# j-wilson/GPflowPILCO

Hardware: AMD Instinct MI355X
Metric: moment_matched_rollout_step_elements_per_sec (higher is better)
Workload: dtype f32; 1 GPU; C3 (BASELINE configs[2]): N=2000 d=8 D=8 H=40 fp32 drift moment-match step / closed rollout; recipe=baseline: BASELINE.md recipe: lengthscales log-U[0.3,3], GP-prior targets, fresh mu~U[0,1]^d / Sigm~; N=2000, d=8, D=8, H=40, B_per_gpu=256, B_total=256, B_this_rank=256, parallelism=dp1 over B (weak), recipe=baseline, steps_requested=418, diag_pairs=f64, offdiag_pairs=f32

## Files before the change

gpflowpilco_amd/_lib.py:

```python
from __future__ import annotations

import ctypes as C
import os

_HERE = os.path.dirname(os.path.abspath(__file__))
LIB_PATH = os.environ.get("GPFLOWPILCO_MM_LIB") or os.path.join(_HERE, "libgpflowpilco_mm.so")

MM_F32, MM_F64 = 0, 1
MM_DMAX = 32
MM_M_ALIGN = 128
MM_FULL_OUTPUT_COV = 1
MM_MODEL_UNCERTAINTY = 2
MM_FORCE_GENERIC = 4
MM_STAGE_DIAG = 8
MM_STAGE_OFFDIAG = 16
MM_STAGE_FINALIZE = 32
MM_FORCE_WORST_TIER = 64
MM_WORKSPACE_CURRENT = 128
MM_FORCE_ROUTE = 256
MM_NO_ROUTE = 512
MM_SUMS_CURRENT = 1024

ERRORS = {
    -1: "MM_E_ARG: NULL pointer or non-positive size",
    -2: "MM_E_DIM: input dimension d exceeds MM_DMAX=32 or unsupported shape",
    -3: "MM_E_DTYPE: dtype must be MM_F32 or MM_F64",
    -4: "MM_E_WORKSPACE: workspace/packed buffer too small",
    -5: "MM_E_NO_C: model_uncertainty requested but the model was packed without C",
    -6: "MM_E_STATE: Euler update / closed rollout needs d == L and a full output covariance",
}

SIGNATURES = {
    "mm_abi_version": (C.c_int, []),
    "mm_packed_model_bytes": (C.c_size_t, [C.c_int] * 5),
    "mm_pack_model": (C.c_int, [C.c_void_p, C.c_size_t, C.c_int, C.c_int, C.c_int, C.c_int]
                      + [C.c_void_p] * 6 + [C.c_void_p]),
    "mm_pack_perm": (C.c_int, [C.c_void_p, C.c_size_t, C.c_int, C.c_int, C.c_int, C.c_int, C.c_void_p, C.c_void_p]),
    "mm_workspace_bytes": (C.c_size_t, [C.c_int] * 6),
    "mm_moment_match": (C.c_int, [C.c_void_p, C.c_size_t, C.c_int, C.c_int, C.c_int, C.c_int, C.c_int,
                                  C.c_void_p, C.c_void_p, C.c_int, C.c_double,
                                  C.c_void_p, C.c_void_p, C.c_void_p,
                                  C.c_void_p, C.c_size_t, C.c_void_p, C.c_void_p]),
    "mm_q_forward": (C.c_int, [C.c_void_p, C.c_size_t, C.c_int, C.c_int, C.c_int, C.c_int, C.c_int,
                               C.c_void_p, C.c_void_p, C.c_int,
                               C.c_void_p, C.c_void_p, C.c_void_p,
                               C.c_void_p, C.c_size_t, C.c_void_p, C.c_void_p]),
    "mm_Q_reduce_forward": (C.c_int, [C.c_void_p, C.c_size_t, C.c_int, C.c_int, C.c_int, C.c_int, C.c_int,
                                      C.c_int, C.c_double, C.c_void_p,
                                      C.c_void_p, C.c_size_t, C.c_void_p]),
    "mm_euler_update": (C.c_int, [C.c_int, C.c_int, C.c_int, C.c_double] + [C.c_void_p] * 8),
    "mm_expected_cost": (C.c_int, [C.c_int, C.c_int, C.c_int] + [C.c_void_p] * 6),
    "mm_offdiag_stats": (C.c_int, [C.c_void_p, C.c_size_t, C.c_int, C.c_int, C.c_int, C.c_int, C.c_int, C.c_int,
                                   C.c_void_p, C.c_size_t, C.c_void_p, C.c_void_p]),
    "mm_route_estimates": (C.c_int, [C.c_void_p, C.c_size_t, C.c_int, C.c_int, C.c_int, C.c_int, C.c_int, C.c_int,
                                     C.c_void_p, C.c_size_t, C.c_void_p, C.c_void_p]),
    "mm_compose_workspace_bytes": (C.c_size_t, [C.c_int] * 4),
    "mm_rollout_composed": (C.c_int, [C.c_void_p, C.c_size_t, C.c_int, C.c_int, C.c_int,
                                      C.c_void_p, C.c_size_t, C.c_int, C.c_int,
                                      C.c_int, C.c_int, C.c_int, C.c_double, C.c_int, C.c_int, C.POINTER(C.c_int32),
                                      C.c_double, C.c_double, C.c_void_p, C.c_void_p,
                                      C.c_void_p, C.c_void_p, C.c_void_p, C.c_void_p, C.c_void_p,
                                      C.c_void_p, C.c_size_t, C.c_void_p, C.c_size_t, C.c_void_p, C.c_size_t,
                                      C.c_void_p, C.c_void_p]),
    "mm_compose_nd_workspace_bytes": (C.c_size_t, [C.c_int] * 5),
    "mm_rollout_composed_nd": (C.c_int, [C.c_void_p, C.c_size_t, C.c_int, C.c_int, C.c_int,
                                         C.c_void_p, C.c_size_t, C.c_int, C.c_int,
                                         C.c_int, C.c_int, C.c_int, C.c_double, C.c_int, C.c_int, C.POINTER(C.c_int32),
                                         C.c_int, C.POINTER(C.c_double), C.POINTER(C.c_double), C.c_void_p, C.c_void_p,
                                         C.c_void_p, C.c_void_p, C.c_void_p, C.c_void_p, C.c_void_p,
                                         C.c_void_p, C.c_size_t, C.c_void_p, C.c_size_t, C.c_void_p, C.c_size_t,
                                         C.c_void_p, C.c_void_p]),
    "mm_compose_tape_bytes": (C.c_size_t, [C.c_int] * 6),
    "mm_rollout_composed_taped": (C.c_int, [C.c_void_p, C.c_size_t, C.c_int, C.c_int, C.c_int,
                                            C.c_void_p, C.c_size_t, C.c_int, C.c_int,
                                            C.c_int, C.c_int, C.c_int, C.c_double, C.c_int, C.c_int, C.POINTER(C.c_int32),
                                            C.c_double, C.c_double, C.c_void_p, C.c_void_p,
                                            C.c_void_p, C.c_void_p, C.c_void_p,
                                            C.c_void_p, C.c_size_t, C.c_void_p, C.c_size_t, C.c_void_p, C.c_size_t,
                                            C.c_void_p, C.c_void_p]),
    "mm_compose_backward_workspace_bytes": (C.c_size_t, [C.c_int] * 4),
    "mm_policy_grad_bytes": (C.c_size_t, [C.c_int] * 3),
    "mm_rollout_composed_backward": (C.c_int, [C.c_void_p, C.c_size_t, C.c_int, C.c_int, C.c_int,
                                               C.c_void_p, C.c_size_t, C.c_int, C.c_int,
                                               C.c_int, C.c_int, C.c_int, C.c_double, C.c_int, C.c_int, C.POINTER(C.c_int32),
                                               C.c_double, C.c_double, C.c_void_p, C.c_void_p,
                                               C.c_void_p, C.c_size_t, C.c_void_p,
                                               C.c_void_p, C.c_void_p, C.c_void_p,
                                               C.c_void_p, C.c_size_t, C.c_void_p, C.c_size_t,
                                               C.c_void_p, C.c_void_p]),
    "mm_rollout_composed_backward_seeded": (C.c_int, [C.c_void_p, C.c_size_t, C.c_int, C.c_int, C.c_int,
                                                      C.c_void_p, C.c_size_t, C.c_int, C.c_int,
                                                      C.c_int, C.c_int, C.c_int, C.c_double, C.c_int, C.c_int, C.POINTER(C.c_int32),
                                                      C.c_double, C.c_double, C.c_void_p, C.c_void_p,
                                                      C.c_void_p, C.c_size_t, C.c_void_p, C.c_void_p, C.c_void_p,
                                                      C.c_void_p, C.c_void_p, C.c_void_p,
                                                      C.c_void_p, C.c_size_t, C.c_void_p, C.c_size_t,
                                                      C.c_void_p, C.c_void_p]),
    "mm_compose_tape_bytes_nd": (C.c_size_t, [C.c_int] * 7),
    "mm_rollout_composed_taped_nd": (C.c_int, [C.c_void_p, C.c_size_t, C.c_int, C.c_int, C.c_int,
                                               C.c_void_p, C.c_size_t, C.c_int, C.c_int,
                                               C.c_int, C.c_int, C.c_int, C.c_double, C.c_int, C.c_int, C.POINTER(C.c_int32),
                                               C.c_int, C.POINTER(C.c_double), C.POINTER(C.c_double), C.c_void_p, C.c_void_p,
                                               C.c_void_p, C.c_void_p, C.c_void_p,
                                               C.c_void_p, C.c_size_t, C.c_void_p, C.c_size_t, C.c_void_p, C.c_size_t,
                                               C.c_void_p, C.c_void_p]),
    "mm_compose_backward_workspace_bytes_nd": (C.c_size_t, [C.c_int] * 6),
    "mm_policy_grad_bytes_nd": (C.c_size_t, [C.c_int] * 4),
    "mm_rollout_composed_backward_nd": (C.c_int, [C.c_void_p, C.c_size_t, C.c_int, C.c_int, C.c_int,
                                                  C.c_void_p, C.c_size_t, C.c_int, C.c_int,
                                                  C.c_int, C.c_int, C.c_int, C.c_double, C.c_int, C.c_int, C.POINTER(C.c_int32),
                                                  C.c_int, C.POINTER(C.c_double), C.POINTER(C.c_double), C.c_void_p, C.c_void_p,
                                                  C.c_void_p, C.c_size_t, C.c_void_p,
                                                  C.c_void_p, C.c_void_p, C.c_void_p,
                                                  C.c_void_p, C.c_size_t, C.c_void_p, C.c_size_t,
                                                  C.c_void_p, C.c_void_p]),
    "mm_rollout_composed_backward_nd_seeded": (C.c_int, [C.c_void_p, C.c_size_t, C.c_int, C.c_int, C.c_int,
                                                         C.c_void_p, C.c_size_t, C.c_int, C.c_int,
                                                         C.c_int, C.c_int, C.c_int, C.c_double, C.c_int, C.c_int, C.POINTER(C.c_int32),
                                                         C.c_int, C.POINTER(C.c_double), C.POINTER(C.c_double), C.c_void_p, C.c_void_p,
                                                         C.c_void_p, C.c_size_t, C.c_void_p, C.c_void_p, C.c_void_p,
                                                         C.c_void_p, C.c_void_p, C.c_void_p,
                                                         C.c_void_p, C.c_size_t, C.c_void_p, C.c_size_t,
                                                         C.c_void_p, C.c_void_p]),
    "mm_compose_nd_mixed_workspace_bytes": (C.c_size_t, [C.c_int] * 6),
    "mm_rollout_composed_nd_mixed": (C.c_int, [C.c_void_p, C.c_size_t, C.c_int, C.c_int, C.c_int,
                                               C.c_void_p, C.c_size_t, C.c_int, C.c_int,
                                               C.c_int, C.c_int, C.c_int, C.c_double, C.c_int, C.c_int, C.POINTER(C.c_int32),
                                               C.c_int, C.POINTER(C.c_double), C.POINTER(C.c_double), C.c_void_p, C.c_void_p,
                                               C.c_void_p, C.c_void_p, C.c_void_p, C.c_void_p, C.c_void_p,
                                               C.c_void_p, C.c_size_t, C.c_void_p, C.c_size_t, C.c_void_p, C.c_size_t,
                                               C.c_void_p, C.c_void_p, C.c_void_p, C.c_void_p]),
    "mm_compose_tape_bytes_nd_mixed": (C.c_size_t, [C.c_int] * 8),
    "mm_rollout_composed_taped_nd_mixed": (C.c_int, [C.c_void_p, C.c_size_t, C.c_int, C.c_int, C.c_int,
                                                     C.c_void_p, C.c_size_t, C.c_int, C.c_int,
                                                     C.c_int, C.c_int, C.c_int, C.c_double, C.c_int, C.c_int, C.POINTER(C.c_int32),
                                                     C.c_int, C.POINTER(C.c_double), C.POINTER(C.c_double), C.c_void_p, C.c_void_p,
# ... 134 lines not shown
```

gpflowpilco_amd/csrc/mm_common.h:

```cpp
#pragma once
#include <stddef.h>
#include <stdint.h>
#include "../../include/gpflowpilco_mm.h"

static inline size_t mm_align_up(size_t x, size_t a) { return (x + a - 1) / a * a; }
static inline int mm_round_up_int(int x, int a) { return (x + a - 1) / a * a; }
static inline size_t mm_elem_size(int dtype) { return dtype == MM_F64 ? 8 : 4; }

#define MM_ISTAGE_NO_ROUTE (1 << 20)
#define MM_ISTAGE_ROUTE (1 << 21)
#define MM_ISTAGE_NO_M56 (1 << 22)
#define MM_ISTAGE_OLD_OFFDIAG (1 << 23)
#define MM_ISTAGE_OLD_SPOLY56 (1 << 24)
#define MM_ISTAGE_OLD_DIAG_MAP (1 << 25)

#define MM_PW_KERNELS 3

static inline int mm_num_pairs(int L, int flags) {
  return (flags & MM_FULL_OUTPUT_COV) ? L * (L + 1) / 2 : L;
}

static inline int mm_moment_deg(int d) { return d <= 8 ? 4 : 2; }
static inline long long mm_binom(int n, int k) {
  if (k < 0 || k > n) return 0;
  long long r = 1;
  for (int i = 1; i <= k; ++i) r = r * (n - k + i) / i;
  return r;
}
static inline int mm_mono_count(int n, int d) { return (int)mm_binom(d + n - 1, n); }
static inline int mm_mono_offset(int n, int d) { int o = 0; for (int m = 0; m < n; ++m) o += mm_mono_count(m, d); return o; }
static inline size_t mm_rank_table_entries(int d) {
  const int dk = d <= 8 ? 8 : 32, deg = mm_moment_deg(d);
  size_t n = 0, p = 1;
  for (int k = 1; k <= deg; ++k) { p *= dk; n += p; }
  return n;
}
static inline int mm_moment_cols(int d) { return mm_round_up_int(mm_mono_offset(mm_moment_deg(d) + 1, d), 16); }
static inline int mm_moment56_off5(int d) { return d <= 8 ? mm_round_up_int(mm_mono_count(4, d), 128) : 0; }
static inline int mm_moment56_off6(int d) { return d <= 8 ? mm_moment56_off5(d) + mm_round_up_int(mm_mono_count(5, d), 128) : 0; }
static inline int mm_moment56_cols(int d) { return d <= 8 ? mm_moment56_off6(d) + mm_round_up_int(mm_mono_count(6, d), 128) : 0; }
struct MMTab56 { int ins[6], last[6], n_i16, mult2, mult3, n_f32; size_t bytes; };
static inline MMTab56 mm_tab56(int d) {
  MMTab56 t;
  int o = 0;
  for (int m = 0; m < 6; ++m) { t.ins[m] = o; o += mm_mono_count(m, d) * 8; }
  for (int k = 0; k < 6; ++k) { t.last[k] = o; o += mm_mono_count(k, d); }
  t.n_i16 = mm_round_up_int(o, 8);
  t.mult2 = 0; t.mult3 = mm_mono_count(2, d); t.n_f32 = mm_mono_count(2, d) + mm_mono_count(3, d);
  t.bytes = (size_t)t.n_i16 * 2 + (size_t)t.n_f32 * 4;
  return t;
}

struct MMModelLayout {
  int Mp, Kz, nd8, KMp;
  size_t Z64;
  size_t Zt64;
  size_t zbar;
  size_t ls2;
  size_t var;
  size_t meanc;
  size_t beta64;
  size_t Zc64;
  size_t Zc;
  size_t Zs3;
  size_t Zm;
  size_t zmax2;
  size_t rtab;
  size_t Zq2;
  size_t Zm56;
  size_t tab56;
  size_t perm;
  size_t skey;
  size_t zt2;
  size_t Cm;
  size_t total;
};
#define MM_SORT_MIN_M 256

static inline MMModelLayout mm_model_layout(int L, int M, int d, int dtype, int with_C) {
  MMModelLayout o;
  const size_t es = mm_elem_size(dtype), A = 256;
  o.Mp = mm_round_up_int(M, MM_M_ALIGN);
  o.Kz = mm_round_up_int(d, 2);
  o.nd8 = (d + 7) / 8;
  o.KMp = mm_moment_cols(d);
  size_t off = 0;
  o.Z64 = off;    off = mm_align_up(off + (size_t)L * M * d * 8, A);
  o.Zt64 = off;   off = mm_align_up(off + (size_t)L * d * o.Mp * 8, A);
  o.zbar = off;   off = mm_align_up(off + (size_t)L * d * 8, A);
  o.ls2 = off;    off = mm_align_up(off + (size_t)L * d * 8, A);
  o.var = off;    off = mm_align_up(off + (size_t)L * 8, A);
  o.meanc = off;  off = mm_align_up(off + (size_t)L * 8, A);
  o.beta64 = off; off = mm_align_up(off + (size_t)L * M * 8, A);
  o.Zc64 = off;   off = mm_align_up(off + (size_t)L * o.Mp * o.Kz * 8, A);
  o.Zc = o.Zc64;
  if (dtype != MM_F64) { o.Zc = off; off = mm_align_up(off + (size_t)L * o.Mp * o.Kz * es, A); }
  o.Zs3 = off;
  if (dtype != MM_F64) off = mm_align_up(off + (size_t)L * o.Mp * 24 * o.nd8 * 2, A);
  o.Zm = off;
  if (dtype != MM_F64) off = mm_align_up(off + (size_t)L * o.Mp * o.KMp * 8, A);
  o.zmax2 = off;  off = mm_align_up(off + (size_t)L * 8, A);
  o.rtab = off;   off = mm_align_up(off + mm_rank_table_entries(d) * 2, A);
  o.Zq2 = off;
  if (dtype != MM_F64 && d <= 8) off = mm_align_up(off + (size_t)L * (o.Mp / 32) * 8192, A);
  o.Zm56 = off;
  if (dtype != MM_F64 && d <= 8) off = mm_align_up(off + (size_t)L * 2 * mm_moment56_cols(d) * o.Mp * 2, A);
  o.tab56 = off;
  if (dtype != MM_F64 && d <= 8) off = mm_align_up(off + mm_tab56(d).bytes, A);
  o.perm = off;   off = mm_align_up(off + (size_t)L * o.Mp * 4, A);
  o.skey = off;   off = mm_align_up(off + (size_t)L * o.Mp * 8, A);
  o.zt2 = off;    off = mm_align_up(off + (size_t)L * (o.Mp / 32) * 4, A);
  o.Cm = off;
  if (with_C) off = mm_align_up(off + (size_t)L * o.Mp * o.Mp * 8, A);
  o.total = off;
  return o;
}

#define MM_MOM_SPLIT 2
#ifndef MM_COLLAPSE_BOUND2
#define MM_COLLAPSE_BOUND2 0.25f
#endif
#define MM_C6_X5_2 (1.0f / 256.0f)
#define MM_C6_X4_2 (1.0f / 1600.0f)
#define MM_C6_MAX 0.25f
#define MM_C6_C0 1.666663289e-01f
#define MM_C6_C1 4.166659713e-02f
#define MM_C6_C2 8.350561373e-03f
#define MM_C6_C3 1.391559141e-03f
#define MM_C6_SYS2 6.33e-6f
#define MM_C6_POLY_F64(x_) (((x_) * (x_)) * (x_) * fma(fma(fma((double)MM_C6_C3, (x_), (double)MM_C6_C2), (x_), (double)MM_C6_C1), (x_), (double)MM_C6_C0))
#ifndef MM_TIER1_DIV
#define MM_TIER1_DIV 20
#endif
#if MM_TIER1_DIV == 16
#define MM_TIER1_MAX 0.0625f
#define MM_REM1_C0 1.666936278e-01f
#define MM_REM1_C1 4.167173430e-02f
#elif MM_TIER1_DIV == 20
#define MM_TIER1_MAX 0.05f
#define MM_REM1_C0 1.666839272e-01f
#define MM_REM1_C1 4.166988656e-02f
#elif MM_TIER1_DIV == 24
#define MM_TIER1_MAX 0.041666668f
#define MM_REM1_C0 1.666786522e-01f
#define MM_REM1_C1 4.166889191e-02f
#elif MM_TIER1_DIV == 32
#define MM_TIER1_MAX 0.03125f
#define MM_REM1_C0 1.666734070e-01f
#define MM_REM1_C1 4.166791216e-02f
#else
#error "MM_TIER1_DIV must be 16, 20, 24 or 32"
#endif
#define MM_INSIDE_BOUND2 (0.998f * MM_C6_MAX * MM_C6_MAX)
#ifndef MM_ROUTE_TOL
#define MM_ROUTE_TOL 3.0e-4
#endif
#define MM_ROUTE_CSPLIT 8
static inline int mm_route_ncc(int NS, int npanel) { int n = NS / npanel; return n < 1 ? 1 : (n > MM_ROUTE_CSPLIT ? MM_ROUTE_CSPLIT : n); }
#define MM_EXP_CAP_F64 700.0
#define MM_EXP_CAP_F32 80.0f
#define MM_GEN_ROWS 64
#define MM_GEN_COLS 256
#define MM_PANEL_ROWS 256
__host__ __device__ inline int mm_mfma_groups(int Mp) { return (Mp + MM_PANEL_ROWS - 1) / MM_PANEL_ROWS * (MM_PANEL_ROWS / 64); }
__host__ __device__ inline int mm_f32p_list_off(int L) { return 4 + 2 * L; }
#define MM_F64_TILE 64

struct MMWorkspaceLayout {
  int Mp, P, Po, NS;
  size_t pairmat;
  size_t latmat;
  size_t rho1;
  size_t w64;
  size_t q64;
  size_t w;
  size_t lq;
  size_t rowD;
  size_t colD;
  size_t qhR;
  size_t qhC;
  size_t rowO;
  size_t colO;
  size_t f1raw;
  size_t whR;
  size_t whC;
  size_t mom;
  size_t amax;
  size_t amaxc;
  size_t gflag;
  size_t gperm;
  size_t s12;
  size_t gmax2;
  size_t partB;
  size_t partC;
  size_t mu64;
  size_t estO;
  size_t rlist;
  size_t rcount;
  size_t rflag;
  size_t wsp;
  size_t mom56;
  size_t estS;
  size_t ilist;
  size_t plist;
  size_t s56;
  size_t f1s;
  size_t Sffs;
  size_t crs;
  size_t total;
};

static inline MMWorkspaceLayout mm_workspace_layout(int B, int L, int M, int d, int dtype, int flags) {
  MMWorkspaceLayout o;
  const size_t es = mm_elem_size(dtype), A = 256;
  o.Mp = mm_round_up_int(M, MM_M_ALIGN);
  o.P = mm_num_pairs(L, flags);
  o.Po = o.P - L;
  const int nrb = (o.Mp + MM_GEN_ROWS - 1) / MM_GEN_ROWS;
  const int ncb = (o.Mp + MM_GEN_COLS - 1) / MM_GEN_COLS;
  const int nt = o.Mp / MM_F64_TILE;
  int ns = nrb * ncb;
  if (nt * (nt + 1) / 2 > ns) ns = nt * (nt + 1) / 2;
  if (dtype == MM_F64 && o.Po > 0 && nt * nt > ns) ns = nt * nt;
  o.NS = ns;
  size_t off = 0;
  o.pairmat = off; off = mm_align_up(off + (size_t)B * o.P * (d * d + 1) * 8, A);
  o.latmat = off;  off = mm_align_up(off + (size_t)B * L * (2 * d * d + 2) * 8, A);
  o.rho1 = off;    off = mm_align_up(off + (size_t)B * L * o.Mp * 8, A);
  o.w64 = off;     off = mm_align_up(off + (size_t)B * L * o.Mp * 8, A);
  o.q64 = off;     off = mm_align_up(off + (size_t)B * L * o.Mp * 8, A);
  o.w = o.w64;
  o.lq = off;      off = mm_align_up(off + (size_t)B * L * o.Mp * 8, A);
  o.rowD = off;    off = mm_align_up(off + (size_t)B * L * o.Mp * 8, A);
  o.colD = off;    off = mm_align_up(off + (size_t)B * L * (d + 1) * o.Mp * 8, A);
  o.qhR = off;     off = mm_align_up(off + (size_t)B * L * o.Mp * 8, A);
  o.qhC = off;     off = mm_align_up(off + (size_t)B * L * o.Mp * 8, A);
  const size_t nrow = dtype == MM_F64 ? 1 : (size_t)(d + 1), ncol = dtype == MM_F64 ? (size_t)(d + 1) : 1;
  o.rowO = off;    off = mm_align_up(off + (size_t)B * o.Po * nrow * o.Mp * es, A);
  o.colO = off;    off = mm_align_up(off + (size_t)B * o.Po * ncol * o.Mp * es, A);
  o.f1raw = off;   off = mm_align_up(off + (size_t)B * L * 8, A);
  const size_t nwh = dtype == MM_F64 ? 0 : (size_t)B * o.Po * o.Mp;
  o.whR = off;     off = mm_align_up(off + nwh * 8, A);
  o.whC = off;     off = mm_align_up(off + nwh * 8, A);
  o.mom = off;     off = mm_align_up(off + (dtype == MM_F64 ? 0 : (size_t)B * o.Po * 2 * MM_MOM_SPLIT * mm_moment_cols(d) * 8), A);
  o.amax = off;    off = off + (size_t)B * o.Po * 4;
  o.amaxc = off;   off = mm_align_up(off + (size_t)B * o.Po * 4, A);
  o.gflag = off;   off = mm_align_up(off + (dtype == MM_F64 ? 0 : (size_t)B * o.Po * (o.Mp / 64)), A);
  o.gmax2 = off;   off = mm_align_up(off + (dtype == MM_F64 ? 0 : (size_t)B * o.Po * (o.Mp / 64) * 4), A);
  o.gperm = off;   off = mm_align_up(off + (dtype == MM_F64 || L < 2 ? 0 : ((size_t)L * (L - 1) * B + 3 * L) * 4), A);
  o.s12 = off;     off = mm_align_up(off + (size_t)B * o.Po * 8, A);
  o.partB = off;   off = mm_align_up(off + (size_t)B * o.P * o.NS * 8, A);
  o.partC = off;   off = mm_align_up(off + (size_t)B * L * o.NS * 8, A);
  const size_t nro = dtype == MM_F64 ? 0 : (size_t)B * o.Po;
  o.mu64 = off;    off = mm_align_up(off + (size_t)B * d * 8, A);
  o.estO = off;    off = mm_align_up(off + nro * ((o.Mp + MM_PANEL_ROWS - 1) / MM_PANEL_ROWS) * 4, A);
  o.rlist = off;   off = mm_align_up(off + nro * 4, A);
  o.rcount = off;  off = mm_align_up(off + 16, A);
  o.rflag = off;   off = mm_align_up(off + nro * 4, A);
  const size_t n56 = (dtype == MM_F64 || d > 8) ? 0 : (size_t)B * o.Po;
  o.wsp = off;     off = mm_align_up(off + n56 * 4 * o.Mp * 2, A);
  o.mom56 = off;   off = mm_align_up(off + n56 * 2 * mm_moment56_cols(d) * 4, A);
  o.estS = off;    off = mm_align_up(off + n56 * 4, A);
  o.s56 = off;     off = mm_align_up(off + n56 * 8, A);
  o.ilist = off;   off = mm_align_up(off + n56 * 4 + 16, A);
  o.plist = off;   off = mm_align_up(off + (n56 ? (n56 + mm_f32p_list_off(L)) * 4 : 0), A);
  o.f1s = off;     off = mm_align_up(off + (size_t)B * L * es, A);
  o.Sffs = off;    off = mm_align_up(off + (size_t)B * L * L * es, A);
  o.crs = off;     off = mm_align_up(off + (size_t)B * d * L * es, A);
  o.total = off;
  return o;
}
```

gpflowpilco_amd/csrc/mm_kernels.hip:

```cpp
#include <hip/hip_runtime.h>
#include <math.h>
#include "mm_common.h"
#include "mm_cost.h"
#include "mm_dev.h"
#include "mm_mono.h"

#include <mutex>
#include <unordered_map>
#include "mm_fork.h"

#define MM_ABI_VERSION 2

namespace {
struct MMForkKey {
  int dev; hipStream_t stream;
  bool operator==(const MMForkKey& o) const { return dev == o.dev && stream == o.stream; }
};
struct MMForkKeyHash {
  size_t operator()(const MMForkKey& k) const { return std::hash<const void*>()((const void*)k.stream) * 31u + (size_t)k.dev; }
};
std::mutex g_fork_mu;
std::unordered_map<MMForkKey, MMFork*, MMForkKeyHash> g_forks;

MMFork* mm_fork_lookup(hipStream_t stream, bool create) {
// ... 107 lines not shown
  const double* Z = (const double*)(packed + lay.Z64);
  double* zbar = (double*)(packed + lay.zbar) + (size_t)a * d;
  double* ls2 = (double*)(packed + lay.ls2) + (size_t)a * d;
  double* Zc64 = (double*)(packed + lay.Zc64) + (size_t)a * lay.Mp * lay.Kz;
  T* Zc = (T*)(packed + lay.Zc) + (size_t)a * lay.Mp * lay.Kz;
  __shared__ double red[4];
  __shared__ double zb[MM_DMAX];
  for (int k = 0; k < d; ++k) {
    double s = 0.0;
    for (int m = tid; m < M; m += 256) s += Z[((size_t)a * M + m) * d + k];
    s = mm_block_sum256(s, red);
    if (tid == 0) zb[k] = s / (double)M;
  }
  __syncthreads();
  if (tid < d) { zbar[tid] = zb[tid]; const double l = ls[a * d + tid]; ls2[tid] = l * l; }
  if (tid == 0) {
    ((double*)(packed + lay.var))[a] = var[a];
    ((double*)(packed + lay.meanc))[a] = mean_c ? mean_c[a] : 0.0;
  }
  {
    double* Zt = (double*)(packed + lay.Zt64) + (size_t)a * d * lay.Mp;
    for (int idx = tid; idx < d * lay.Mp; idx += 256) {
      const int k = idx / lay.Mp, m = idx - k * lay.Mp;
      Zt[idx] = m < M ? Z[((size_t)a * M + m) * d + k] : 0.0;
    }
  }
  for (int idx = tid; idx < lay.Mp * lay.Kz; idx += 256) {
    const int m = idx / lay.Kz, k = idx - m * lay.Kz;
    double v = 0.0;
    if (m < M && k < d) v = Z[((size_t)a * M + m) * d + k] - zb[k];
    Zc64[idx] = v;
    if (sizeof(T) != 8) Zc[idx] = (T)v;
  }
  if (sizeof(T) != 8) {
    double* Zm = (double*)(packed + lay.Zm) + (size_t)a * lay.Mp * lay.KMp;
    const int deg = d <= 8 ? 4 : 2;
    const int ncol = mm_mono_off(deg + 1, d);
    for (int idx = tid; idx < lay.Mp * lay.KMp; idx += 256) {
      const int m = idx / lay.KMp, c = idx - m * lay.KMp;
      double v = 0.0;
      if (m < M && c < ncol) {
        int n = 0;
        while (mm_mono_off(n + 1, d) <= c) ++n;
        int k[4] = {0, 0, 0, 0};
        mm_mono_unrank(c - mm_mono_off(n, d), n, k);
        v = 1.0;
        for (int t = 0; t < n; ++t) v *= Z[((size_t)a * M + m) * d + k[t]] - zb[k[t]];
      }
      Zm[idx] = v;
    }
    if (a == 0) {
      short* rt = (short*)(packed + lay.rtab);
      const int lb = d <= 8 ? 3 : 5;
      size_t base = 0;
      for (int kk = 1; kk <= deg; ++kk) {
        const int sz = 1 << (lb * kk);
        for (int idx = tid; idx < sz; idx += 256) {
          int dg[4] = {0, 0, 0, 0};
          bool in = true;
          for (int t = 0; t < kk; ++t) { dg[t] = (idx >> (lb * t)) & ((1 << lb) - 1); in = in && dg[t] < d; }
          for (int i = 1; i < kk; ++i)
            for (int j = i; j > 0 && dg[j - 1] > dg[j]; --j) { const int t2 = dg[j]; dg[j] = dg[j - 1]; dg[j - 1] = t2; }
          rt[base + idx] = in ? (short)mm_mono_rank(dg, kk) : (short)-1;
        }
        base += sz;
      }
    }
  }
  {
    double zm2 = 0.0;
    for (int m = tid; m < M; m += 256) {
      double s2 = 0.0;
      for (int k = 0; k < d; ++k) { const double v = Z[((size_t)a * M + m) * d + k] - zb[k]; s2 += v * v; }
      zm2 = s2 > zm2 ? s2 : zm2;
    }
#pragma unroll
    for (int off = 32; off > 0; off >>= 1) { const double o = __shfl_down(zm2, off, 64); zm2 = o > zm2 ? o : zm2; }
    __syncthreads();
    if ((tid & 63) == 0) red[tid >> 6] = zm2;
    __syncthreads();
    if (tid == 0) ((double*)(packed + lay.zmax2))[a] = fmax(fmax(red[0], red[1]), fmax(red[2], red[3]));
    __syncthreads();
    float* zt2 = (float*)(packed + lay.zt2) + (size_t)a * (lay.Mp / 32);
    for (int t = tid; t < lay.Mp / 32; t += 256) {
      double mx = 0.0;
      for (int j = 0; j < 32; ++j) {
        const int m = t * 32 + j;
        if (m >= M) break;
        double s2 = 0.0;
        for (int k = 0; k < d; ++k) { const double v = Z[((size_t)a * M + m) * d + k] - zb[k]; s2 += v * v; }
        mx = s2 > mx ? s2 : mx;
      }
      zt2[t] = (float)(mx * 1.000001);
    }
  }
  if (sizeof(T) != 8) {
    unsigned short* Zs3 = (unsigned short*)(packed + lay.Zs3) + (size_t)a * lay.Mp * 24 * lay.nd8;
    const int kw = 8 * lay.nd8;
    for (int idx = tid; idx < lay.Mp * kw; idx += 256) {
      const int m = idx / kw, k = idx - m * kw;
      float v = 0.0f;
      if (m < M && k < d) v = (float)(Z[((size_t)a * M + m) * d + k] - zb[k]);
      const __bf16 h = (__bf16)v;
      float r = v - (float)h;
      const __bf16 mm = (__bf16)r;
      r -= (float)mm;
      const __bf16 l = (__bf16)r;
      unsigned short* o = Zs3 + ((size_t)(m >> 5) * 3 * 32 + (m & 31)) * kw + k;
      o[0] = __builtin_bit_cast(unsigned short, h);
      o[32 * kw] = __builtin_bit_cast(unsigned short, mm);
      o[64 * kw] = __builtin_bit_cast(unsigned short, l);
    }
    if (d <= 8) {
      unsigned short* Zq = (unsigned short*)(packed + lay.Zq2) + (size_t)a * (lay.Mp / 32) * 4096;
      const int nslot = 1 + d + d * (d + 1) / 2;
      for (int idx = tid; idx < (lay.Mp / 32) * 2048; idx += 256) {
        int r = idx;
        const int t = r & 7; r >>= 3;
        const int ln = r & 63; r >>= 6;
        const int nb = r & 1; r >>= 1;
        const int s2 = r & 1; r >>= 1;
        const int ct = r;
        const int slot = 32 * nb + (ln & 31), hh = ln >> 5;
        const int m = 32 * ct + 16 * s2 + 8 * (t >> 2) + 4 * hh + (t & 3);
        float v = 0.0f;
        if (m < M && slot < nslot) {
          if (slot == 0) v = 1.0f;
          else if (slot <= d) v = (float)(Z[((size_t)a * M + m) * d + slot - 1] - zb[slot - 1]);
          else {
            int qq = slot - 1 - d, l0 = 0;
            while (qq >= d - l0) { qq -= d - l0; ++l0; }
            const int l1 = l0 + qq;
            v = (float)((Z[((size_t)a * M + m) * d + l0] - zb[l0]) * (Z[((size_t)a * M + m) * d + l1] - zb[l1]));
          }
        }
        const __bf16 h = (__bf16)v;
        const __bf16 lo = (__bf16)(v - (float)h);
        unsigned short* o = Zq + ((((size_t)(ct * 2 + s2) * 2 + nb) * 2) * 64 + ln) * 8 + t;
        o[0] = __builtin_bit_cast(unsigned short, h);
        o[512] = __builtin_bit_cast(unsigned short, lo);
      }
    }
  }
}

__global__ void k_pack_C(char* packed, MMModelLayout lay, int L, int M, const double* __restrict__ C) {
  const int j = blockIdx.x * 256 + threadIdx.x, i = blockIdx.y, a = blockIdx.z;
  if (j >= lay.Mp) return;
  double* Cm = (double*)(packed + lay.Cm) + ((size_t)a * lay.Mp + i) * lay.Mp;
  const int* pm = (const int*)(packed + lay.perm) + (size_t)a * lay.Mp;
  double v = 0.0;
  if (i < M && j < M) v = C[((size_t)a * M + pm[i]) * M + pm[j]];
  Cm[j] = v;
}

template <typename T>
__global__ __launch_bounds__(192) void k_prep(const double* __restrict__ ls2, const double* __restrict__ var,
                                              int L, int d, int P,
                                              const T* __restrict__ mu, const T* __restrict__ Sigma,
                                              double* __restrict__ pairmat, double* __restrict__ latmat,
                                              unsigned int* __restrict__ amax, int32_t* status, int pairs_pass) {
  extern __shared__ double smem[];
  const int dp = d + 1, msz = d * dp;
  double* Sg = smem;
  double* A0 = Sg + msz;
  double* A1 = A0 + msz;
  double* A2 = A1 + msz;
  double* Tm = A2 + msz;
  double* Y = Tm + msz;
  __shared__ double lds3[3];
  __shared__ int okw[3];
  const int tid = threadIdx.x, nt = blockDim.x, wv = tid >> 6;
  const int item = pairs_pass == 0 ? P + blockIdx.x : blockIdx.x, b = blockIdx.y;
  bool ok = true;
  const T* Sb = Sigma + (size_t)b * d * d;
  for (int idx = tid; idx < d * d; idx += nt) {
// ... 179 lines not shown
        maha = fma(z[i], t, maha);
        rv = fma(z[i], te, rv);
      };
      if constexpr (QREG) {
        int t = 0;
#pragma unroll
        for (int i = 0; i < DK; ++i) {
          const double pd = Pr[QREG ? t : 0] * z[i], ed = Er[QREG ? t : 0] * z[i];
          ++t;
          double tp = 0.0, te = 0.0;
#pragma unroll
          for (int k = i + 1; k < DK; ++k, ++t) { tp = fma(Pr[QREG ? t : 0], z[k], tp); te = fma(Er[QREG ? t : 0], z[k], te); }
          maha = fma(z[i], fma(2.0, tp, pd), maha);
          rv = fma(z[i], fma(2.0, te, ed), rv);
        }
      } else {
#pragma unroll 2
        for (int i = 0; i < DK; ++i) row(i);
      }
      lqv = lognorm - 0.5 * maha;
      qv = exp(lqv);
      wv = bt * qv;
      acc_f += wv;
#pragma unroll
      for (int k = 0; k < DK; ++k) acc_s[k] += wv * z[k];
      if (q_out) q_out[((size_t)b * L + a) * M + perm[(size_t)a * Mp + m]] = (T)qv;
    }
    wb64[m] = wv;
    qb64[m] = qv;
    r1[m] = rv;
    lqb[m] = lqv;
  };
  {
    double zA[DK], zB[DK], bA, bB;
    loadz(tid, zA, bA);
    for (int m = tid; m < Mp; m += 512) {
      loadz(m + 256 < Mp ? m + 256 : m, zB, bB);
      chunk(m, zA, bA);
      if (m + 256 >= Mp) break;
      loadz(m + 512 < Mp ? m + 512 : m + 256, zA, bA);
      chunk(m + 256, zB, bB);
    }
  }
  __shared__ double red9[4][DK + 1];
  {
    double v[DK + 1];
#pragma unroll
    for (int k = 0; k < DK; ++k) v[k] = acc_s[k];
    v[DK] = acc_f;
#pragma unroll
    for (int k = 0; k <= DK; ++k) {
#pragma unroll
      for (int off = 32; off > 0; off >>= 1) v[k] += __shfl_down(v[k], off, 64);
    }
    if ((tid & 63) == 0) {
#pragma unroll
      for (int k = 0; k <= DK; ++k) red9[tid >> 6][k] = v[k];
    }
  }
  __syncthreads();
  if (tid <= DK) sv[tid] = (red9[0][tid] + red9[1][tid]) + (red9[2][tid] + red9[3][tid]);
  __syncthreads();
  if (tid == 0) { f1[(size_t)b * L + a] = (T)(sv[DK] + meanc[a]); f1raw[(size_t)b * L + a] = sv[DK]; }
  if (tid < d) {
    double s = 0.0;
    for (int k = 0; k < d; ++k) s += Pa[tid * DK + k] * sv[k];
    cross[((size_t)b * d + tid) * L + a] = (T)s;
  }
}

template <typename T, int DK>
__global__ __launch_bounds__(256) void k_pairvec(const double* __restrict__ Zt64, const double* __restrict__ zbar,
                                                 const double* __restrict__ ls2, int L, int M, int Mp, int d, int P,
                                                 const T* __restrict__ mu, const double* __restrict__ pairmat,
                                                 const double* __restrict__ rho1,
                                                 double* __restrict__ rowD, double* __restrict__ colD,
                                                 T* __restrict__ rowO, T* __restrict__ colO,
                                                 const double* __restrict__ w64, double* __restrict__ whR,
                                                 double* __restrict__ whC, unsigned int* __restrict__ amax,
                                                 const double* __restrict__ q64, double* __restrict__ qhR,
                                                 double* __restrict__ qhC, int with_unc, int nblk,
                                                 const double* __restrict__ lq, const double* __restrict__ beta64,
                                                 const double* __restrict__ zmax2, unsigned short* __restrict__ ,
                                                 unsigned char* __restrict__ , float* __restrict__ , int , int p0) {
  static_assert(DK > 8, "d <= 8 takes k_pairvec_reg");
  const int p = p0 + (int)blockIdx.y, b = blockIdx.z, tid = threadIdx.x;
  int a, a2;
  mm_decode_pair(p, L, a, a2);
  const double* r1a = rho1 + ((size_t)b * L + a) * Mp;
  const double* r1b = rho1 + ((size_t)b * L + a2) * Mp;
  __shared__ __align__(16) double Ts[DK * DK];
  __shared__ double vecs[7][DK];
  __shared__ int rcs;
  const double* pm = pairmat + ((size_t)b * P + p) * (d * d + 1);
  for (int idx = tid; idx < DK * DK; idx += 256) {
    const int i = idx / DK, k = idx - i * DK;
    const bool in = i < d && k < d;
    Ts[idx] = in ? pm[i * d + k] * ls2[a * d + i] * ls2[a2 * d + k] : 0.0;
  }
  if (tid < DK) {
    const int k = tid < d ? tid : 0;
    const double mv = (double)mu[(size_t)b * d + k];
    const double la = ls2[a * d + k], lb = ls2[a2 * d + k];
    vecs[0][tid] = tid < d ? mv : 0.0;
    vecs[1][tid] = tid < d ? 1.0 / la : 0.0;
    vecs[2][tid] = tid < d ? 1.0 / lb : 0.0;
    vecs[3][tid] = tid < d ? (mv - zbar[a2 * d + k]) / lb : 0.0;
    vecs[4][tid] = tid < d ? (mv - zbar[a * d + k]) / la : 0.0;
  }
  __syncthreads();
  const double cst = pm[d * d];
  const bool diag = p < L;
  const int Po = P - L;
  const bool f32off = !diag && sizeof(T) == 4;
  if (f32off) {
    if (tid < DK) {
      double t = 0.0;
      for (int k = 0; k < DK; ++k) t = fma(Ts[tid * DK + k], vecs[4][k], t);
      vecs[5][tid] = t;
    }
    __syncthreads();
    if (tid == 0) {
      double sa2 = 0.0, c00 = 0.0;
      for (int i = 0; i < DK; ++i) { const double sa = vecs[5][i] * vecs[2][i]; sa2 = fma(sa, sa, sa2); c00 = fma(vecs[5][i], vecs[3][i], c00); }
      const bool rc = sa2 * zmax2[a2] <= MM_RECENTRE_CMAX * MM_RECENTRE_CMAX;
      rcs = rc ? 1 : 0;
      vecs[6][0] = rc ? c00 : 0.0;
      if (!rc) for (int i = 0; i < DK; ++i) vecs[5][i] = 0.0;
    }
    __syncthreads();
  }
  const bool recentred = f32off ? rcs != 0 : true;
  T* rO = rowO + ((size_t)b * Po + (f32off ? p - L : 0)) * (size_t)(d + 1) * Mp;
  T* cO = colO + ((size_t)b * Po + (f32off ? p - L : 0)) * Mp;
  double* hR = whR + ((size_t)b * Po + (f32off ? p - L : 0)) * Mp;
  double* hC = whC + ((size_t)b * Po + (f32off ? p - L : 0)) * Mp;
  double* raD = rowD + ((size_t)b * L + (diag ? p : 0)) * Mp;
  double* cbD = colD + ((size_t)b * L + (diag ? p : 0)) * (size_t)(d + 1) * Mp;
  T* raO = rowO + ((size_t)b * Po + (diag ? 0 : p - L)) * Mp;
  T* cbO = colO + ((size_t)b * Po + (diag ? 0 : p - L)) * (size_t)(d + 1) * Mp;
  float a2max = 0.0f;
  for (int mblk = blockIdx.x; mblk < nblk; mblk += gridDim.x) {
    const int m = mblk * 256 + tid;
    if (m >= Mp) continue;
    typedef const __attribute__((address_space(3))) double* lds_cptr;
    lds_cptr vl = (lds_cptr)&vecs[0][0], tl = (lds_cptr)Ts;
    asm volatile("" : "+v"(vl), "+v"(tl));
    double zr[DK], zc[DK];
#pragma unroll
    for (int k = 0; k < DK; ++k) {
      const int kk = k < d ? k : 0;
      const double vr = Zt64[((size_t)a * d + kk) * Mp + m];
      const double vc = Zt64[((size_t)a2 * d + kk) * Mp + m];
      zr[k] = (m < M) ? (vr - vl[k]) * vl[DK + k] : 0.0;
      zc[k] = (m < M) ? (vc - vl[k]) * vl[2 * DK + k] : 0.0;
    }
    const double r1r = r1a[m], r1c = r1b[m];
    const int mc = m < M ? m : M - 1;
    const double lqr = lq[((size_t)b * L + a) * Mp + m], lqc = lq[((size_t)b * L + a2) * Mp + m];
    const double btr = beta64[(size_t)a * M + mc], btc = beta64[(size_t)a2 * M + mc];
    double tA = 0.0, tg = 0.0, corrA = 0.0, corrg = 0.0;
    double asq = 0.0, cj = vl[6 * DK];
#pragma unroll 2
    for (int i = 0; i < DK; ++i) {
      double u = 0.0, v = 0.0;
#pragma unroll
      for (int k = 0; k < DK; ++k) {
        const double t = tl[i * DK + k];
        u = fma(t, zr[k], u);
        v = fma(t, zc[k], v);
      }
      tA = fma(zr[i], u, tA);
      tg = fma(zc[i], v, tg);
      corrA = fma(vl[3 * DK + i], u, corrA);
      corrg = fma(vl[4 * DK + i], v, corrg);
      const double t0i = f32off ? vl[5 * DK + i] : 0.0;
      cj = fma(t0i, zc[i], cj);
      const double av = (u + t0i) * vl[2 * DK + i], gv = v * vl[DK + i];
      asq = fma(av, av, asq);
      if (i < d) {
        if (f32off) rO[(size_t)i * Mp + m] = (T)av;
        else if (diag) cbD[(size_t)i * Mp + m] = gv;
        else cbO[(size_t)i * Mp + m] = (T)gv;
      }
    }
    const double rho_q = (m < M) ? r1r - tA : 0.0;
    const double gam_q = (m < M) ? r1c - tg : 0.0;
    if (f32off) {
      a2max = fmaxf(a2max, (float)asq * 1.000001f);
      double whr = 0.0, whc = 0.0;
      if (m < M) {
        whr = btr * exp(fmin(lqr - 0.5 * rho_q + cst - corrA, (double)MM_EXP_CAP_F32));
        whc = btc * exp(fmin(lqc - 0.5 * gam_q - cj, (double)MM_EXP_CAP_F32));
      }
      rO[(size_t)d * Mp + m] = (T)whr;
      cO[m] = (T)whc;
      hR[m] = whr;
      hC[m] = whc;
    } else {
      const double rowv = -0.5 * rho_q;
      const double colv = (m < M) ? -0.5 * gam_q + cst - corrg : 0.0;
      if (diag) {
        raD[m] = rowv; cbD[(size_t)d * Mp + m] = colv;
        const size_t qi = ((size_t)b * L + p) * Mp + m;
        const double u = (m < M) ? (with_unc ? 1.0 : btr) : 0.0;
        qhR[qi] = u * exp(fmin(lqr + rowv, MM_EXP_CAP_F64));
        qhC[qi] = u * exp(fmin(lqr + colv, MM_EXP_CAP_F64));
      } else { raO[m] = (T)rowv; cbO[(size_t)d * Mp + m] = (T)colv; }
    }
  }
  if (f32off && amax) {
#pragma unroll
    for (int off = 32; off > 0; off >>= 1) a2max = fmaxf(a2max, __shfl_down(a2max, off, 64));
    if ((tid & 63) == 0) atomicMax(amax + (size_t)b * Po + (p - L), recentred ? __float_as_uint(a2max) : MM_AMAX_NOT_RECENTRED);
  }
}

template <typename T, int DK, int MODE>
__device__ __forceinline__ void mm_pairvec_reg_body(const double* __restrict__ Zt64, const double* __restrict__ zbar,
                                                    const double* __restrict__ ls2, int L, int M, int Mp, int d, int P,
                                                    const T* __restrict__ mu, const double* __restrict__ pairmat,
                                                    const double* __restrict__ rho1,
                                                    double* __restrict__ rowD, double* __restrict__ colD,
                                                    T* __restrict__ rowO, T* __restrict__ colO,
                                                    const double* __restrict__ w64, double* __restrict__ whR,
                                                    double* __restrict__ whC, unsigned int* __restrict__ amax,
                                                    const double* __restrict__ q64, double* __restrict__ qhR,
                                                    double* __restrict__ qhC, int with_unc, int nblk, int a, int a2,
                                                    double (*vecs)[DK], const double* __restrict__ lq,
                                                    const double* __restrict__ beta64, int p, const double* __restrict__ zmax2,
                                                    unsigned short* __restrict__ wsp, unsigned char* __restrict__ gflag, float* __restrict__ gmax2,
                                                    int allow) {
  constexpr bool diag = MODE == 0;
  const int b = blockIdx.z, tid = threadIdx.x;
  const int Po = P - L;
  const double* zA = Zt64 + (size_t)a * d * Mp;
  const double* zB = Zt64 + (size_t)a2 * d * Mp;
  const double* r1a = rho1 + ((size_t)b * L + a) * Mp;
  const double* r1b = rho1 + ((size_t)b * L + a2) * Mp;
  const double* wa = lq + ((size_t)b * L + a) * Mp;
  const double* wb = lq + ((size_t)b * L + a2) * Mp;
  const double* ba = beta64 + (size_t)a * M;
  const double* bb = beta64 + (size_t)a2 * M;
  struct Ops { double zr[DK], zc[diag ? 1 : DK], r1r, r1c, wr, wc, br, bc; };
  auto load_ops = [&](int mblk, Ops& o) {
    int m = mblk * 256 + tid;
    m = m < Mp ? m : Mp - 1;
#pragma unroll
    for (int k = 0; k < DK; ++k) {
      const unsigned off = (unsigned)((k < d ? k : 0) * Mp + m);
      o.zr[k] = zA[off];
      if constexpr (!diag) o.zc[k] = zB[off];
    }
    o.r1r = r1a[m];
    o.wr = wa[m];
    const int mb = m < M ? m : M - 1;
    o.br = ba[mb];
    if constexpr (!diag) { o.r1c = r1b[m]; o.wc = wb[m]; o.bc = bb[mb]; }
  };
  Ops oA, oB;
  load_ops(blockIdx.x, oA);
  const double* pm = pairmat + ((size_t)b * P + p) * (d * d + 1);
  constexpr int NT = DK * (DK + 1) / 2;
  double Tr[NT];
  auto tsym = [](int i, int k) { return i <= k ? i * DK - i * (i - 1) / 2 + (k - i) : k * DK - k * (k - 1) / 2 + (i - k); };
  {
    const int ln = tid & 63, li = ln / DK, lk = ln - li * DK;
    const bool lin = li < d && lk < d && ln < DK * DK;
    const double mine = lin ? pm[li * d + lk] * ls2[a * d + li] * ls2[a2 * d + lk] : 0.0;
    const int mlo = __double2loint(mine), mhi = __double2hiint(mine);
#pragma unroll
    for (int i = 0; i < DK; ++i)
#pragma unroll
      for (int k = i; k < DK; ++k) {
        double t = __hiloint2double(__builtin_amdgcn_readlane(mhi, i * DK + k), __builtin_amdgcn_readlane(mlo, i * DK + k));
        asm volatile("" : "+v"(t));
        Tr[tsym(i, k)] = t;
      }
  }
  if (tid < DK) {
    const int k = tid < d ? tid : 0;
    const double mv = (double)mu[(size_t)b * d + k];
    const double la = ls2[a * d + k], lb = ls2[a2 * d + k];
    vecs[0][tid] = tid < d ? mv : 0.0;
    vecs[1][tid] = tid < d ? 1.0 / la : 0.0;
    vecs[2][tid] = tid < d ? 1.0 / lb : 0.0;
    vecs[3][tid] = tid < d ? (mv - zbar[a2 * d + k]) / lb : 0.0;
    vecs[4][tid] = tid < d ? (mv - zbar[a * d + k]) / la : 0.0;
  }
  __syncthreads();
  bool recentred = true;
  if constexpr (MODE == 0) {
    double h2 = 0.0, t0[DK];
#pragma unroll
    for (int i = 0; i < DK; ++i) {
      double t = 0.0;
#pragma unroll
      for (int k = 0; k < DK; ++k) t = fma(Tr[tsym(i, k)], vecs[4][k], t);
      t0[i] = t;
      const double hi = t * vecs[1][i];
      h2 = fma(hi, hi, h2);
    }
    recentred = h2 * zmax2[a] <= MM_RECENTRE_CMAX * MM_RECENTRE_CMAX;
    if (tid == 0) {
#pragma unroll
      for (int i = 0; i < DK; ++i) vecs[5][i] = recentred ? t0[i] : 0.0;
    }
    __syncthreads();
  }
  if constexpr (MODE == 1) {
    double sa2 = 0.0, c00 = 0.0, t0[DK];
#pragma unroll
    for (int i = 0; i < DK; ++i) {
      double t = 0.0;
#pragma unroll
      for (int k = 0; k < DK; ++k) t = fma(Tr[tsym(i, k)], vecs[4][k], t);
      t0[i] = t;
      const double sa = t * vecs[2][i];
      sa2 = fma(sa, sa, sa2);
      c00 = fma(t, vecs[3][i], c00);
    }
    recentred = sa2 * zmax2[a2] <= MM_RECENTRE_CMAX * MM_RECENTRE_CMAX;
    if (tid == 0) {
#pragma unroll
      for (int i = 0; i < DK; ++i) vecs[5][i] = recentred ? t0[i] : 0.0;
      vecs[6][0] = recentred ? c00 : 0.0;
    }
    __syncthreads();
  }
  const double cst = pm[d * d];
  float a2max = 0.0f;
  float a2cmax = 0.0f, a2in = 0.0f;
  const bool cancoll = MODE == 1 && allow && recentred;
  const double zm2c = MODE == 1 ? zmax2[a2] : 0.0;
  typedef const __attribute__((address_space(3))) double* lds_cptr;
  auto rowi = [&](int i) { return (unsigned)((i < d ? i : d) * Mp); };
  const unsigned rowd = (unsigned)(d * Mp);

  auto body = [&](int mblk, const Ops& o) {
    const int m = mblk * 256 + tid;
    if (m >= Mp) return;
    lds_cptr vl = (lds_cptr)&vecs[0][0];
    asm volatile("" : "+v"(vl));
    const bool live = m < M;
    if constexpr (MODE == 0) {
      double* cbD = colD + ((size_t)b * L + p) * (size_t)(d + 1) * Mp;
      double* raD = rowD + ((size_t)b * L + p) * Mp;
      double* qR = qhR + ((size_t)b * L + p) * Mp;
      double* qC = qhC + ((size_t)b * L + p) * Mp;
      if (live) {
        double sv[DK];
#pragma unroll
        for (int k = 0; k < DK; ++k) sv[k] = (o.zr[k] - vl[k]) * vl[DK + k];
        double tq = 0.0, corr = 0.0, zh = 0.0;
#pragma unroll
        for (int i = 0; i < DK; ++i) {
          double u = 0.0;
#pragma unroll
          for (int k = 0; k < DK; ++k) u = fma(Tr[tsym(i, k)], sv[k], u);
          tq = fma(sv[i], u, tq);
          corr = fma(vl[4 * DK + i], u, corr);
          zh = fma(sv[i] + vl[4 * DK + i], vl[5 * DK + i], zh);
          cbD[rowi(i) + m] = (u + vl[5 * DK + i]) * vl[DK + i];
        }
        const double row0 = -0.5 * (o.r1r - tq);
        const double rowv = row0 - zh;
        const double colv = row0 + cst - corr;
        const double uw = with_unc ? 1.0 : o.br;
        raD[m] = rowv; cbD[rowd + m] = colv;
        qR[m] = uw * exp(fmin(o.wr + rowv, MM_EXP_CAP_F64)); qC[m] = uw * exp(fmin(o.wr + colv, MM_EXP_CAP_F64));
      } else {
#pragma unroll
        for (int i = 0; i < DK; ++i) cbD[rowi(i) + m] = 0.0;
        raD[m] = 0.0; cbD[rowd + m] = 0.0; qR[m] = 0.0; qC[m] = 0.0;
      }
    } else if constexpr (MODE == 1) {
      T* rO = rowO + ((size_t)b * Po + (p - L)) * (size_t)(d + 1) * Mp;
      T* cO = colO + ((size_t)b * Po + (p - L)) * Mp;
      double* hR = whR + ((size_t)b * Po + (p - L)) * Mp;
      double* hC = whC + ((size_t)b * Po + (p - L)) * Mp;
      double whr = 0.0, whc = 0.0;
      bool rowok = true;
      if (live) {
        double sr[DK], sc[DK];
        double cj = vl[6 * DK];
#pragma unroll
        for (int k = 0; k < DK; ++k) {
          const double muk = vl[k];
          sr[k] = (o.zr[k] - muk) * vl[DK + k]; sc[k] = (o.zc[k] - muk) * vl[2 * DK + k];
          cj = fma(vl[5 * DK + k], sc[k], cj);
        }
        double tA = 0.0, tg = 0.0, corrA = 0.0, asq = 0.0;
#pragma unroll
        for (int i = 0; i < DK; ++i) {
          double u = 0.0, vh = 0.0;
#pragma unroll
          for (int k = 0; k < DK; ++k) {
            const double t = Tr[tsym(i, k)];
            u = fma(t, sr[k], u);
            if (k > i) vh = fma(t, sc[k], vh);
          }
          tA = fma(sr[i], u, tA);
          tg = fma(sc[i], fma(2.0, vh, Tr[tsym(i, i)] * sc[i]), tg);
          const double av = (u + vl[5 * DK + i]) * vl[2 * DK + i];
          asq = fma(av, av, asq);
          corrA = fma(vl[3 * DK + i], u, corrA);
          rO[rowi(i) + m] = (T)av;
        }
        const float a2row = (float)asq * 1.000001f;
        a2max = fmaxf(a2max, a2row);
        rowok = mm_collapse_bound2(__float_as_uint(a2row), zm2c) <= MM_COLLAPSE_BOUND2;
        a2in = a2row;
        whr = o.br * exp(fmin(o.wr - 0.5 * (o.r1r - tA) + cst - corrA, (double)MM_EXP_CAP_F32));
        whc = o.bc * exp(fmin(o.wc - 0.5 * (o.r1c - tg) - cj, (double)MM_EXP_CAP_F32));
      } else {
#pragma unroll
        for (int i = 0; i < DK; ++i) rO[rowi(i) + m] = (T)0;
        a2in = 0.0f;
      }
      rO[rowd + m] = (T)whr; cO[m] = (T)whc; hR[m] = whr; hC[m] = whc;
      if (wsp) {
        const bool inner = cancoll && __all(rowok);
        float g2 = a2in;
#pragma unroll
        for (int off = 32; off > 0; off >>= 1) g2 = fmaxf(g2, __shfl_xor(g2, off, 64));
        if ((tid & 63) == 0) {
          const size_t gi = ((size_t)b * Po + (p - L)) * (size_t)(Mp / MM_GROUP_ROWS) + (m >> 6);
          gflag[gi] = inner ? 1 : 0;
          gmax2[gi] = g2;
        }
        if (inner) a2cmax = fmaxf(a2cmax, a2in);
        unsigned short* sp = wsp + ((size_t)b * Po + (p - L)) * 4 * (size_t)Mp + m;
        const float fr = inner ? (float)whr : 0.0f, fc = (float)whc;
        const __bf16 rh = (__bf16)fr, ch = (__bf16)fc;
        const __bf16 rm = (__bf16)(fr - (float)rh), cm = (__bf16)(fc - (float)ch);
        sp[0] = __builtin_bit_cast(unsigned short, rh); sp[Mp] = __builtin_bit_cast(unsigned short, rm);
        sp[2 * (size_t)Mp] = __builtin_bit_cast(unsigned short, ch); sp[3 * (size_t)Mp] = __builtin_bit_cast(unsigned short, cm);
      }
    } else {
      T* raO = rowO + ((size_t)b * Po + (p - L)) * Mp;
      T* cbO = colO + ((size_t)b * Po + (p - L)) * (size_t)(d + 1) * Mp;
      if (live) {
        double sr[DK], sc[DK];
#pragma unroll
        for (int k = 0; k < DK; ++k) { const double muk = vl[k]; sr[k] = (o.zr[k] - muk) * vl[DK + k]; sc[k] = (o.zc[k] - muk) * vl[2 * DK + k]; }
        double tA = 0.0, tg = 0.0, corrg = 0.0;
#pragma unroll
        for (int i = 0; i < DK; ++i) {
          double v = 0.0, uh = 0.0;
#pragma unroll
          for (int k = 0; k < DK; ++k) {
            const double t = Tr[tsym(i, k)];
            v = fma(t, sc[k], v);
            if (k > i) uh = fma(t, sr[k], uh);
          }
          tg = fma(sc[i], v, tg);
          tA = fma(sr[i], fma(2.0, uh, Tr[tsym(i, i)] * sr[i]), tA);
          corrg = fma(vl[4 * DK + i], v, corrg);
          cbO[rowi(i) + m] = (T)(v * vl[DK + i]);
        }
        raO[m] = (T)(-0.5 * (o.r1r - tA));
        cbO[rowd + m] = (T)(-0.5 * (o.r1c - tg) + cst - corrg);
      } else {
#pragma unroll
        for (int i = 0; i < DK; ++i) cbO[rowi(i) + m] = (T)0;
        raO[m] = (T)0; cbO[rowd + m] = (T)0;
      }
    }
  };

  const int step = (int)gridDim.x;
  for (int mblk = blockIdx.x; mblk < nblk; mblk += 2 * step) {
    load_ops(mblk + step < nblk ? mblk + step : mblk, oB);
    body(mblk, oA);
    if (mblk + step >= nblk) break;
    load_ops(mblk + 2 * step < nblk ? mblk + 2 * step : mblk + step, oA);
    body(mblk + step, oB);
  }
  if (MODE == 1 && amax) {
#pragma unroll
    for (int off = 32; off > 0; off >>= 1) a2max = fmaxf(a2max, __shfl_down(a2max, off, 64));
    if ((tid & 63) == 0) atomicMax(amax + (size_t)b * Po + (p - L), recentred ? __float_as_uint(a2max) : MM_AMAX_NOT_RECENTRED);
#pragma unroll
    for (int off = 32; off > 0; off >>= 1) a2cmax = fmaxf(a2cmax, __shfl_down(a2cmax, off, 64));
    if ((tid & 63) == 0 && a2cmax > 0.0f) atomicMax(amax + ((size_t)gridDim.z + b) * Po + (p - L), __float_as_uint(a2cmax));
  }
}

template <typename T, int DK>
__global__ __launch_bounds__(256, 2) void k_pairvec_reg(const double* __restrict__ Zt64, const double* __restrict__ zbar,
                                                        const double* __restrict__ ls2, int L, int M, int Mp, int d, int P,
                                                        const T* __restrict__ mu, const double* __restrict__ pairmat,
                                                        const double* __restrict__ rho1,
                                                        double* __restrict__ rowD, double* __restrict__ colD,
                                                        T* __restrict__ rowO, T* __restrict__ colO,
                                                        const double* __restrict__ w64, double* __restrict__ whR,
                                                        double* __restrict__ whC, unsigned int* __restrict__ amax,
                                                        const double* __restrict__ q64, double* __restrict__ qhR,
                                                        double* __restrict__ qhC, int with_unc, int nblk,
                                                        const double* __restrict__ lq, const double* __restrict__ beta64,
                                                        const double* __restrict__ zmax2, unsigned short* __restrict__ wsp,
                                                        unsigned char* __restrict__ gflag, float* __restrict__ gmax2, int allow, int p0) {
  static_assert(DK <= 8, "register form: d <= 8");
  __shared__ double vecs[7][DK];
  const int p = p0 + (int)blockIdx.y;
  int a, a2;
  mm_decode_pair(p, L, a, a2);
#define MM_PV_BODY(MODE_)                                                                                           \
  mm_pairvec_reg_body<T, DK, MODE_>(Zt64, zbar, ls2, L, M, Mp, d, P, mu, pairmat, rho1, rowD, colD, rowO, colO, w64, \
                                    whR, whC, amax, q64, qhR, qhC, with_unc, nblk, a, a2, vecs, lq, beta64, p, zmax2, wsp, gflag, gmax2, allow)
  if (p < L) MM_PV_BODY(0);
  else if (sizeof(T) == 4) MM_PV_BODY(1);
  else MM_PV_BODY(2);
#undef MM_PV_BODY
}

template <typename T, int DK, bool ROWVEC>
__global__ __launch_bounds__(256) void k_qred_generic(const T* __restrict__ Zc, int Kz, const double* __restrict__ Cm,
                                                      int L, int Mp, int d, int P, int NS, int ncb, int p0,
                                                      const T* __restrict__ w, const T* __restrict__ q,
                                                      const T* __restrict__ rowA, const T* __restrict__ colB,
                                                      double* __restrict__ partB, double* __restrict__ partC,
                                                      const unsigned char* __restrict__ gflag, const unsigned int* __restrict__ amaxc,
                                                      const double* __restrict__ zmax2) {
  const int cbk = blockIdx.x % ncb, rbk = blockIdx.x / ncb;
  const int lp = blockIdx.y, np = gridDim.y, p = p0 + lp, b = blockIdx.z, tid = threadIdx.x;
  int a, a2;
  mm_decode_pair(p, L, a, a2);
  const int j = cbk * MM_GEN_COLS + tid;
  const bool jv = j < Mp;
  const int jj = jv ? j : 0;
  const T* cb = ROWVEC ? colB + ((size_t)b * np + lp) * Mp
                       : colB + ((size_t)b * np + lp) * (size_t)(d + 1) * Mp;
  T g[DK];
#pragma unroll
  for (int k = 0; k < DK; ++k)
    g[k] = (k < d) ? (ROWVEC ? Zc[((size_t)a2 * Mp + jj) * Kz + k] : cb[(size_t)k * Mp + jj]) : (T)0;
  const T gam = ROWVEC ? (T)0 : cb[(size_t)d * Mp + jj];
  const T wj = jv ? (ROWVEC ? cb[jj] : w[((size_t)b * L + a2) * Mp + jj]) : (T)0;
  const bool withC = (Cm != nullptr) && (a == a2);
  const T qj = (withC && jv) ? q[((size_t)b * L + a2) * Mp + jj] : (T)0;
  const T* ra = ROWVEC ? rowA + ((size_t)b * np + lp) * (size_t)(d + 1) * Mp
                       : rowA + ((size_t)b * np + lp) * Mp;
  const T* wr = w + ((size_t)b * L + a) * Mp;
  const T* qr = q + ((size_t)b * L + a) * Mp;
  const T* zrow = Zc + (size_t)a * Mp * Kz;
  const int i0 = rbk * MM_GEN_ROWS;
  const int i1 = (i0 + MM_GEN_ROWS < Mp) ? i0 + MM_GEN_ROWS : Mp;
  T accB = (T)0;
  double sumB = 0.0, sumC = 0.0;
  const unsigned char* gf = (ROWVEC && gflag != nullptr && zmax2 != nullptr) ? gflag + ((size_t)b * np + lp) * (size_t)(Mp / MM_GROUP_ROWS) : nullptr;
  const bool icoll = gf != nullptr && mm_item_collapsed(amaxc[(size_t)b * np + lp]);
  for (int i = i0; i < i1; ++i) {
    const bool coll = icoll && gf[i >> 6] != 0;
    T delta = ROWVEC ? (T)0 : ra[i] + gam;
#pragma unroll
    for (int k = 0; k < DK; ++k)
      if (k < d) delta += (ROWVEC ? ra[(size_t)k * Mp + i] : zrow[(size_t)i * Kz + k]) * g[k];
    const double dd = fmin((double)delta, sizeof(T) == 8 ? MM_EXP_CAP_F64 : (double)MM_EXP_CAP_F32);
    const T e = ROWVEC ? (T)(expm1(dd) - dd - 0.5 * dd * dd - (coll ? MM_C6_POLY_F64(dd) : (icoll ? (double)MM_C6_C0 * dd * dd * dd : 0.0)))
                       : (T)expm1(dd);
    accB += (ROWVEC ? ra[(size_t)d * Mp + i] : wr[i]) * e;
    if (withC) {
      const double cij = Cm[((size_t)a * Mp + i) * Mp + jj];
      const double qi = (double)qr[i];
      sumC += cij * (qi * (double)e + qi);
    }
    if (((i - i0) & 15) == 15) { sumB += (double)accB; accB = (T)0; }
  }
  sumB += (double)accB;
  sumB *= (double)wj;
  sumC *= (double)qj;
  __shared__ double red[4];
  const double tb = mm_block_sum256(sumB, red);
  if (tid == 0) partB[((size_t)b * P + p) * NS + blockIdx.x] = tb;
  if (withC) {
    const double tc = mm_block_sum256(sumC, red);
    if (tid == 0) partC[((size_t)b * L + a) * NS + blockIdx.x] = tc;
  }
}

template <typename T>
__global__ __launch_bounds__(256) void k_finalize(const double* __restrict__ partB, const double* __restrict__ partC,
                                                  const double* __restrict__ var, int B, int L, int P, int NS,
                                                  int nsB_diag, int nsB_off, int nsC, int full, int with_unc,
                                                  double jitter, const double* __restrict__ f1raw,
                                                  const double* __restrict__ s12, const double* __restrict__ s56, int diag_factored,
                                                  const int* __restrict__ rflag, int ns_routed, T* __restrict__ Sff) {
  const int idx = blockIdx.x * 4 + (threadIdx.x >> 6), lane = threadIdx.x & 63;
  if (idx >= B * P) return;
  const int b = idx / P, p = idx - b * P;
  int a, a2;
  mm_decode_pair(p, L, a, a2);
// ... 125 lines not shown
  hipLaunchKernelGGL(k_pack_gather, dim3((M + 255) / 256, L), dim3(256), 0, s, packed, lay, M, d, Z, beta);
  MM_CHECK_LAUNCH();
  hipLaunchKernelGGL((k_pack_vectors<T>), dim3(L), dim3(256), 0, s, packed, lay, L, M, d, ls, var, mean_c);
  MM_CHECK_LAUNCH();
  if (sizeof(T) == 4 && d <= 8) {
    const int rc = mm_launch_pack56(packed, lay, L, M, d, (const double*)(packed + lay.Z64), s);
    if (rc) return rc;
  }
  if (C) {
    hipLaunchKernelGGL(k_pack_C, dim3((lay.Mp + 255) / 256, lay.Mp, L), dim3(256), 0, s, packed, lay, L, M, C);
    MM_CHECK_LAUNCH();
  }
  return 0;
}

extern "C" int mm_pack_model(void* packed, size_t packed_bytes, int L, int M, int d, int dtype,
                             const double* Z, const double* lengthscales, const double* variance,
                             const double* beta, const double* C, const double* mean_c, void* stream) {
  int rc = mm_check_common(packed, L, M, d, dtype, 1);
  if (rc) return rc;
  if (!Z || !lengthscales || !variance || !beta) return MM_E_ARG;
  const MMModelLayout lay = mm_model_layout(L, M, d, dtype, C != nullptr);
  if (packed_bytes < lay.total) return MM_E_WORKSPACE;
  hipStream_t s = (hipStream_t)stream;
  if (dtype == MM_F64) return mm_pack_model_t<double>((char*)packed, lay, L, M, d, Z, lengthscales, variance, beta, C, mean_c, s);
  return mm_pack_model_t<float>((char*)packed, lay, L, M, d, Z, lengthscales, variance, beta, C, mean_c, s);
}

extern "C" int mm_pack_perm(const void* packed, size_t packed_bytes, int L, int M, int d, int dtype, int32_t* perm, void* stream) {
  int rc = mm_check_common(packed, L, M, d, dtype, 1);
  if (rc) return rc;
  if (!perm) return MM_E_ARG;
  const MMModelLayout lay = mm_model_layout(L, M, d, dtype, 0);
  if (packed_bytes < lay.total) return MM_E_WORKSPACE;
  const hipError_t e = hipMemcpy2DAsync(perm, (size_t)M * 4, (const char*)packed + lay.perm, (size_t)lay.Mp * 4, (size_t)M * 4, (size_t)L,
                                        hipMemcpyDeviceToDevice, (hipStream_t)stream);
  return e == hipSuccess ? 0 : (int)e;
}

template <typename T, int DK>
static int mm_q_forward_t(const char* packed, const MMModelLayout& ml, char* ws, const MMWorkspaceLayout& wl,
                          int L, int M, int d, int B, const T* mu, const T* Sigma, int flags,
                          T* f1, T* cross, T* q_out, int32_t* status, hipStream_t s, bool joins) {
  const double* ls2 = (const double*)(packed + ml.ls2);
  const double* var = (const double*)(packed + ml.var);
  const double* Z64 = (const double*)(packed + ml.Z64);
  double* pairmat = (double*)(ws + wl.pairmat);
  double* latmat = (double*)(ws + wl.latmat);
  const size_t shm = (size_t)8 * d * (d + 1) * sizeof(double);
  unsigned int* amax = (sizeof(T) == 4 && wl.Po > 0) ? (unsigned int*)(ws + wl.amax) : nullptr;
  if ((long long)(wl.P + L) * B <= 4096) {
    hipLaunchKernelGGL((k_prep<T>), dim3(wl.P + L, B), dim3(192), shm, s,
                       ls2, var, L, d, wl.P, mu, Sigma, pairmat, latmat, amax, status, 2);
    MM_CHECK_LAUNCH();
  } else {
    hipLaunchKernelGGL((k_prep<T>), dim3(L, B), dim3(64), shm, s,
                       ls2, var, L, d, wl.P, mu, Sigma, pairmat, latmat, amax, status, 0);
    MM_CHECK_LAUNCH();
    hipLaunchKernelGGL((k_prep<T>), dim3(wl.P, B), dim3(64), shm, s,
                       ls2, var, L, d, wl.P, mu, Sigma, pairmat, latmat, amax, status, 1);
    MM_CHECK_LAUNCH();
  }
  hipLaunchKernelGGL((k_qvec<T, DK>), dim3(L, B), dim3(256), 0, s,
                     (const double*)(packed + ml.Zt64), (const double*)(packed + ml.beta64), (const double*)(packed + ml.meanc),
                     L, M, wl.Mp, d, mu, latmat, (double*)(ws + wl.w64), (double*)(ws + wl.q64), (T*)(ws + wl.w),
                     (double*)(ws + wl.f1raw), (double*)(ws + wl.rho1), f1, cross, q_out, (double*)(ws + wl.mu64), (double*)(ws + wl.lq),
                     (const int*)(packed + ml.perm));
  MM_CHECK_LAUNCH();
  {
    const int nblk = (wl.Mp + 255) / 256;
    auto nsplit_for = [&](int npairs) {
      long long per = (long long)npairs * B;
      int ns = (int)((4096 + per - 1) / per);
      if (ns > nblk) ns = nblk;
      return ns < 1 ? 1 : ns;
    };
#define MM_PAIRVEC_ARGS                                                                                                     \
    (const double*)(packed + ml.Zt64), (const double*)(packed + ml.zbar), ls2, L, M, wl.Mp, d, wl.P, mu, pairmat,            \
    (const double*)(ws + wl.rho1), (double*)(ws + wl.rowD), (double*)(ws + wl.colD), (T*)(ws + wl.rowO), (T*)(ws + wl.colO), \
    (const double*)(ws + wl.w64), (double*)(ws + wl.whR), (double*)(ws + wl.whC), amax,                                      \
    (const double*)(ws + wl.q64), (double*)(ws + wl.qhR), (double*)(ws + wl.qhC), (flags & MM_MODEL_UNCERTAINTY) ? 1 : 0, nblk, \
    (const double*)(ws + wl.lq), (const double*)(packed + ml.beta64), (const double*)(packed + ml.zmax2),                       \
    ((sizeof(T) == 4 && d <= 8) ? (unsigned short*)(ws + wl.wsp) : (unsigned short*)nullptr),                                \
    (unsigned char*)(ws + wl.gflag), (float*)(ws + wl.gmax2), ((flags & (MM_FORCE_WORST_TIER | MM_ISTAGE_NO_M56)) ? 0 : 1)
    auto pairvec = [&](int p0, int npairs, hipStream_t st) {
      if (npairs <= 0) return;
      if constexpr (DK <= 8) {
        hipLaunchKernelGGL((k_pairvec_reg<T, DK>), dim3(nsplit_for(npairs), npairs, B), dim3(256), 0, st, MM_PAIRVEC_ARGS, p0);
      } else {
        hipLaunchKernelGGL((k_pairvec<T, DK>), dim3(nsplit_for(npairs), npairs, B), dim3(256), 0, st, MM_PAIRVEC_ARGS, p0);
      }
    };
    pairvec(0, L, s);
    MM_CHECK_LAUNCH();
    if (wl.Po > 0) {
      MMFork* fork = (joins && (long long)wl.P * B >= 512) ? mm_fork_get(s) : nullptr;
      hipStream_t s2 = s;
      if (fork) {
        hipError_t ef = hipEventRecord(fork->fork, s);
        if (ef == hipSuccess) ef = hipStreamWaitEvent(fork->s2, fork->fork, 0);
        if (ef != hipSuccess) return (int)ef;
        s2 = fork->s2;
      }
      pairvec(L, wl.Po, s2);
      int rcs = 0;
      { hipError_t e_ = hipGetLastError(); if (e_ != hipSuccess) rcs = (int)e_; }
      if (!rcs && sizeof(T) == 4) rcs = mm_launch_moments(packed, ml, ws, wl, B, L, d, (const void*)mu, flags, s2);
      if (fork) {
        hipError_t ej = hipEventRecord(fork->join, fork->s2);
        if (rcs) { if (ej == hipSuccess) (void)hipStreamWaitEvent(s, fork->join, 0); return rcs; }
        if (ej != hipSuccess) return (int)ej;
      }
      if (rcs) return rcs;
    }
#undef MM_PAIRVEC_ARGS
  }
  MM_CHECK_LAUNCH();
  return 0;
}

template <typename T, int DK>
static int mm_Q_reduce_t(const char* packed, const MMModelLayout& ml, bool has_C, char* ws, const MMWorkspaceLayout& wl,
                         int L, int M, int d, int B, int flags, double jitter, T* Sff, int32_t* status, hipStream_t s) {
  const int with_unc = (flags & MM_MODEL_UNCERTAINTY) ? 1 : 0;
  const int full = (flags & MM_FULL_OUTPUT_COV) ? 1 : 0;
  if (with_unc && !has_C) return MM_E_NO_C;
  const double* Cm = with_unc ? (const double*)(packed + ml.Cm) : nullptr;
  double* partB = (double*)(ws + wl.partB);
  double* partC = (double*)(ws + wl.partC);
  const int nrb = (wl.Mp + MM_GEN_ROWS - 1) / MM_GEN_ROWS, ncb = (wl.Mp + MM_GEN_COLS - 1) / MM_GEN_COLS;
  const bool generic = (flags & MM_FORCE_GENERIC) != 0;
  const bool use_mfma32 = sizeof(T) == 4 && !generic && mm_mfma_supported(d);
  const int ns_gen = nrb * ncb;
  const int nsB_diag = generic ? ns_gen : mm_f64_num_slots(wl.Mp, 1), nsC = nsB_diag;
  const int nsB_off = generic ? ns_gen : (sizeof(T) == 4 ? (use_mfma32 ? mm_mfma_num_slots(wl.Mp) : ns_gen)
                                                         : mm_f64_num_slots(wl.Mp, 0));
  int stages = flags & (MM_STAGE_DIAG | MM_STAGE_OFFDIAG | MM_STAGE_FINALIZE);
  if (!stages) stages = MM_STAGE_DIAG | MM_STAGE_OFFDIAG | MM_STAGE_FINALIZE;
  const bool routes = use_mfma32 && wl.Po > 0 && !(flags & (MM_FORCE_WORST_TIER | MM_NO_ROUTE));
  bool both = false;
  if (sizeof(T) == 8 && !generic && wl.Po > 0 && (stages & (MM_STAGE_DIAG | MM_STAGE_OFFDIAG)) == (MM_STAGE_DIAG | MM_STAGE_OFFDIAG)) {
    if (const int rj = mm_fork_join_wait(s)) return rj;
    const int rc = mm_launch_qred_f64_both((const double*)(packed + ml.Zc64), ml.Kz, Cm, (const double*)(packed + ml.beta64), M, L,
                                           wl.Mp, d, wl.P, wl.NS, wl.Po, B, (flags & MM_FORCE_WORST_TIER) ? 1 : 0,
                                           (const double*)(ws + wl.qhR), (const double*)(ws + wl.qhC), (const double*)(ws + wl.rowD),
                                           (const double*)(ws + wl.colD), (const double*)(ws + wl.w64), (const double*)(ws + wl.q64),
                                           (const double*)(ws + wl.rowO), (const double*)(ws + wl.colO), partB, partC, s, &both);
    if (rc) return rc;
  }
  if (!both && (stages & MM_STAGE_DIAG)) {
    if (generic) {
      hipLaunchKernelGGL((k_qred_generic<double, DK, false>), dim3(nrb * ncb, L, B), dim3(256), 0, s,
                         (const double*)(packed + ml.Zc64), ml.Kz, Cm, L, wl.Mp, d, wl.P, wl.NS, ncb, 0,
                         (const double*)(ws + wl.w64), (const double*)(ws + wl.q64),
                         (const double*)(ws + wl.rowD), (const double*)(ws + wl.colD), partB, partC,
                         (const unsigned char*)nullptr, (const unsigned int*)nullptr, (const double*)nullptr);
      MM_CHECK_LAUNCH();
    } else {
      const int rc = mm_launch_qred_f64((const double*)(packed + ml.Zc64), ml.Kz, Cm,
                                        (const double*)(packed + ml.beta64), M, L, wl.Mp, d, wl.P, wl.NS,
                                        0, L, B, 1, sizeof(T) == 4 ? 1 : 0, (flags & MM_FORCE_WORST_TIER) ? 1 : 0,
                                        (flags & MM_ISTAGE_OLD_DIAG_MAP) ? 1 : 0,
                                        (const double*)(ws + wl.qhR), (const double*)(ws + wl.qhC),
                                        (const double*)(ws + wl.rowD), (const double*)(ws + wl.colD),
                                        partB, partC, s);
      if (rc) return rc;
    }
// ... 198 lines not shown
```

gpflowpilco_amd/csrc/mm_mfma.hip:

```cpp
#include <hip/hip_runtime.h>
#include <math.h>
#include <atomic>
#include "mm_common.h"
#include "mm_mono.h"
#include "mm_f32_tile.h"

__device__ __forceinline__ void mm_decode_pair_o(int p, int L, int& a, int& a2) {
  int r = p - L, i = 0;
  while (r >= L - 1 - i) { r -= L - 1 - i; ++i; }
  a = i; a2 = i + 1 + r;
}

#ifndef MM_TWO_WAY_MAX
#define MM_TWO_WAY_MAX 0.03125f
#endif
#ifndef MM_F32_PPW_DIV
#define MM_F32_PPW_DIV 2
#endif
#ifndef MM_ROUTE_EST
#define MM_ROUTE_EST 1
#endif
#ifndef MM_F32_WAVES
#define MM_F32_WAVES 2
#endif
template <int DEG, int CC>
struct MMRemC {
  static constexpr float get(int k) {
    const float c6[4] = {MM_C6_C0, MM_C6_C1, MM_C6_C2, MM_C6_C3};
    return MMRem<DEG>::c[k] - ((CC == 1 && k < 4) ? c6[k] : ((CC == 2 && k == 0) ? c6[0] : 0.0f));
  }
};
template <int DEG, int CC>
__device__ __forceinline__ f32x2 mm_weighted_rem(const f32x2 (&xx)[16], const f32x2 (&wrow)[2][8]) {
  f32x2 parts[4] = {{0.f, 0.f}, {0.f, 0.f}, {0.f, 0.f}, {0.f, 0.f}};
#pragma unroll
  for (int hh = 0; hh < 2; ++hh) {
    f32x2 pp[8];
#pragma unroll
    for (int r = 0; r < 8; ++r)
      pp[r] = mm_pkfma(MM_PK((MMRemC<DEG, CC>::get(DEG))), xx[8 * hh + r], MM_PK((MMRemC<DEG, CC>::get(DEG - 1))));
#pragma unroll
    for (int k = DEG - 2; k >= 0; --k)
#pragma unroll
      for (int r = 0; r < 8; ++r)
        pp[r] = mm_pkfma(pp[r], xx[8 * hh + r], MM_PK((MMRemC<DEG, CC>::get(k))));
#pragma unroll
    for (int r = 0; r < 8; ++r) {
      const f32x2 wx = wrow[hh][r] * xx[8 * hh + r];
      const f32x2 tv = (xx[8 * hh + r] * xx[8 * hh + r]) * pp[r];
      parts[r & 3] = mm_pkfma(tv, wx, parts[r & 3]);
    }
  }
  return (parts[0] + parts[1]) + (parts[2] + parts[3]);
}

__device__ __forceinline__ f32x2 mm_weighted_rem1(const f32x2 (&xx)[16], const f32x2 (&wc0)[2][8],
                                                  const f32x2 (&wc1)[2][8]) {
  f32x2 parts[4] = {{0.f, 0.f}, {0.f, 0.f}, {0.f, 0.f}, {0.f, 0.f}};
#pragma unroll
  for (int hh = 0; hh < 2; ++hh) {
    f32x2 t3[8], rw[8];
#pragma unroll
    for (int r = 0; r < 8; ++r) t3[r] = xx[8 * hh + r] * xx[8 * hh + r];
#pragma unroll
    for (int r = 0; r < 8; ++r) rw[r] = mm_pkfma(wc1[hh][r], xx[8 * hh + r], wc0[hh][r]);
#pragma unroll
    for (int r = 0; r < 8; ++r) t3[r] = t3[r] * xx[8 * hh + r];
#pragma unroll
    for (int r = 0; r < 8; ++r) parts[r & 3] = mm_pkfma(t3[r], rw[r], parts[r & 3]);
  }
  return (parts[0] + parts[1]) + (parts[2] + parts[3]);
}

template <int ND8, bool LDSZ>
__global__ __launch_bounds__(256, (ND8 >= 4 ? 1 : MM_F32_WAVES)) void k_qred_f32_mfma(const unsigned short* __restrict__ Zs3,
                                                          int L, int Mp, int d, int P, int Po, int NS,
                                                          int npanel, int ppw, int nwork, int force_worst,
                                                          const unsigned int* __restrict__ amax,
                                                          const unsigned int* __restrict__ amaxc,
                                                          const unsigned char* __restrict__ gflag, const float* __restrict__ gmax2,
                                                          const double* __restrict__ zmax2, const float* __restrict__ zt2,
                                                          const float* __restrict__ rowO,
                                                          const float* __restrict__ colO,
                                                          double* __restrict__ partB, float* __restrict__ estO,
                                                          int* __restrict__ rcount) {
  const int orig = blockIdx.x;
  if (orig == 0 && threadIdx.x == 0 && rcount) { rcount[0] = 0; rcount[1] = 0; }
  const int xcd = orig & 7, slot = orig >> 3;
  const int qn = nwork >> 3, rn = nwork & 7;
  const int wi = (xcd < rn ? xcd * (qn + 1) : rn * (qn + 1) + (xcd - rn) * qn) + slot;
  const int npw = (npanel + ppw - 1) / ppw;
  const int pgrp = wi % npw;
  const int t = wi / npw;
  const int lp = t % Po, b = t / Po;
  const int p = L + lp;
  int a, a2;
  mm_decode_pair_o(p, L, a, a2);

  const int wv = threadIdx.x >> 6, lane = threadIdx.x & 63, l31 = lane & 31, h = lane >> 5;
  if constexpr (ND8 == 1) {
    if (!force_worst && zmax2 && mm_collapse_bound2(amax[(size_t)b * Po + lp], zmax2[a2]) <= MM_INSIDE_BOUND2) {
      for (int panel = (int)threadIdx.x; panel < npanel; panel += 256) {
        if (panel % npw != pgrp) continue;
        partB[((size_t)b * P + p) * NS + panel] = 0.0;
        if (estO) estO[((size_t)b * Po + lp) * npanel + panel] = 0.0f;
      }
      return;
    }
  }
  const bool icoll_wg = (ND8 == 1) && !force_worst && zmax2 != nullptr && zt2 != nullptr && gmax2 != nullptr &&
                        mm_item_collapsed(amaxc[(size_t)b * Po + lp]);
  const size_t grp0 = ((size_t)b * Po + lp) * (size_t)(Mp / MM_GROUP_ROWS);
  if constexpr (ND8 == 1) {
    if (icoll_wg) {
      bool need = false;
      for (int panel = pgrp; panel < npanel; panel += npw) {
        const int g = (panel * MM_PANEL_ROWS + wv * 64) >> 6;
        if (g < Mp / MM_GROUP_ROWS)
          need = need || !(gflag[grp0 + g] != 0 && mm_collapse_bound2(__float_as_uint(gmax2[grp0 + g]), zmax2[a2]) <= MM_INSIDE_BOUND2);
      }
      if (!__syncthreads_or(need ? 1 : 0)) {
        for (int panel = (int)threadIdx.x; panel < npanel; panel += 256) {
          if (panel % npw != pgrp) continue;
          partB[((size_t)b * P + p) * NS + panel] = 0.0;
          if (estO) estO[((size_t)b * Po + lp) * npanel + panel] = 0.0f;
        }
        return;
      }
    }
  }
  extern __shared__ __align__(16) char zlds[];
  if constexpr (LDSZ) {
    const char* src = reinterpret_cast<const char*>(Zs3 + (size_t)a2 * Mp * (24 * ND8));
    const int nchunk = (Mp >> 5) * 64 * ND8;
    for (int c0 = 0; c0 < nchunk; c0 += 8 * 256) {
      u32x4 tmp[8];
#pragma unroll
      for (int u = 0; u < 8; ++u) {
        int c = c0 + u * 256 + (int)threadIdx.x;
        c = c < nchunk ? c : nchunk - 1;
        const int tile = c / (64 * ND8), within = c - tile * (64 * ND8);
        tmp[u] = *reinterpret_cast<const u32x4*>(src + (size_t)tile * (1536 * ND8) + (size_t)within * 16);
      }
#pragma unroll
      for (int u = 0; u < 8; ++u) {
        const int c = c0 + u * 256 + (int)threadIdx.x;
        if (c < nchunk) *reinterpret_cast<u32x4*>(zlds + (size_t)c * 16) = tmp[u];
      }
    }
    __syncthreads();
  }
  __shared__ double red[4];
  __shared__ float redf[4];
  for (int panel = pgrp; panel < npanel; panel += npw) {
  const int row0 = panel * MM_PANEL_ROWS + wv * 64;
  double sum = 0.0;
  f32x2 est2 = {0.0f, 0.0f};
  float rowsq = 0.0f, xall = 0.0f;
  const bool icoll = icoll_wg;
  const bool coll = icoll && row0 < Mp && gflag[grp0 + (row0 >> 6)] != 0;
  const float g2 = coll ? gmax2[grp0 + (row0 >> 6)] : 0.0f;
  const bool wave_inside = coll && mm_collapse_bound2(__float_as_uint(g2), zmax2[a2]) <= MM_INSIDE_BOUND2;
  if (row0 < Mp && !wave_inside) {
    const float* ra = rowO + ((size_t)b * Po + lp) * (size_t)(d + 1) * Mp;
    const float* wcf = colO + ((size_t)b * Po + lp) * Mp;
    const unsigned short* zs = Zs3 + (size_t)a2 * Mp * (24 * ND8);
    const float bound2 = zmax2 ? mm_collapse_bound2(amaxc[(size_t)b * Po + lp], zmax2[a2]) : 3.0e38f;
    const float thr_skip = MM_C6_MAX - 0.00390625f * __builtin_sqrtf(bound2) - 1e-6f;

    bf16x8 a1[2][ND8], a2v[2][ND8], a3[2][ND8];
    f32x2 wrow[2][8], wc0[2][8], wc1[2][8];
#pragma unroll
    for (int rt = 0; rt < 2; ++rt) {
      const int row = row0 + rt * 32 + l31;
#pragma unroll
      for (int nb = 0; nb < ND8; ++nb) {
        unsigned int hh[8], mm[8], ll[8];
#pragma unroll
        for (int j = 0; j < 8; ++j) {
          const int k = nb * 8 + j;
          const float v = ra[(size_t)(k < d ? k : d) * Mp + row];
          mm_split3(k < d ? v : 0.0f, hh[j], mm[j], ll[j]);
        }
        u32x4 ph, pm, pl;
#pragma unroll
        for (int j = 0; j < 4; ++j) {
          ph[j] = hh[2 * j] | (hh[2 * j + 1] << 16);
          pm[j] = mm[2 * j] | (mm[2 * j + 1] << 16);
          pl[j] = ll[2 * j] | (ll[2 * j + 1] << 16);
        }
        a1[rt][nb] = __builtin_bit_cast(bf16x8, pm);
        a2v[rt][nb] = __builtin_bit_cast(bf16x8, h ? pl : ph);
        a3[rt][nb] = __builtin_bit_cast(bf16x8, ph);
      }
#pragma unroll
      for (int g = 0; g < 4; ++g) {
        const int rr = row0 + rt * 32 + 8 * g + 4 * h;
        const float4 v = *reinterpret_cast<const float4*>(ra + (size_t)d * Mp + rr);
        wrow[rt][2 * g + 0] = (f32x2){v.x, v.y};
        wrow[rt][2 * g + 1] = (f32x2){v.z, v.w};
        if constexpr (ND8 == 1) {
#pragma unroll
          for (int q2 = 0; q2 < 2; ++q2) {
            wc0[rt][2 * g + q2] = wrow[rt][2 * g + q2] * MM_PK(MMRem<1>::c[0]);
            wc1[rt][2 * g + q2] = wrow[rt][2 * g + q2] * MM_PK(MMRem<1>::c[1]);
          }
        }
      }
    }
    {
      f32x2 rs = {0.0f, 0.0f};
#pragma unroll
      for (int rt = 0; rt < 2; ++rt)
#pragma unroll
        for (int r = 0; r < 8; ++r) rs = mm_pkfma(wrow[rt][r], wrow[rt][r], rs);
      rowsq = rs[0] + rs[1];
    }

    const unsigned int tile_bytes = 32u * 48u * ND8, part_bytes = 32u * 16u * ND8;
    const unsigned int offA = (h ? 0u : 1u) * part_bytes + (unsigned int)l31 * (16u * ND8);
    const unsigned int offB = (h ? 0u : 2u) * part_bytes + (unsigned int)l31 * (16u * ND8);
    const char* zbase = reinterpret_cast<const char*>(zs);
    const int nct = Mp >> 5;

    auto load_zA = [&](int ct, u32x4 (&zA)[ND8]) {
#pragma unroll
      for (int nb = 0; nb < ND8; ++nb) {
        if constexpr (LDSZ) zA[nb] = *reinterpret_cast<const u32x4*>(zlds + (size_t)ct * (1024 * ND8) + offA + nb * 16);
        else zA[nb] = *reinterpret_cast<const u32x4*>(zbase + (size_t)ct * tile_bytes + offA + nb * 16);
      }
    };
    auto load_zB = [&](int ct, u32x4 (&zB)[ND8]) {
#pragma unroll
      for (int nb = 0; nb < ND8; ++nb) zB[nb] = *reinterpret_cast<const u32x4*>(zbase + (size_t)ct * tile_bytes + offB + nb * 16);
    };

    auto mfma_tile_screen = [&](const u32x4 (&zA)[ND8], f32x16 (&acc)[2]) {
#pragma unroll
      for (int rt = 0; rt < 2; ++rt) {
        f32x16 c = {0.f, 0.f, 0.f, 0.f, 0.f, 0.f, 0.f, 0.f, 0.f, 0.f, 0.f, 0.f, 0.f, 0.f, 0.f, 0.f};
#pragma unroll
        for (int nb = 0; nb < ND8; ++nb)
          c = __builtin_amdgcn_mfma_f32_32x32x16_bf16(a3[rt][nb], __builtin_bit_cast(bf16x8, zA[nb]), c, 0, 0, 0);
        acc[rt] = c;
      }
// ... 1 lines not shown
    auto mfma_tile_m = [&](const u32x4 (&zA)[ND8], f32x16 (&acc)[2]) {
#pragma unroll
      for (int rt = 0; rt < 2; ++rt) {
        f32x16 c = acc[rt];
#pragma unroll
        for (int nb = 0; nb < ND8; ++nb)
          c = __builtin_amdgcn_mfma_f32_32x32x16_bf16(a1[rt][nb], __builtin_bit_cast(bf16x8, zA[nb]), c, 0, 0, 0);
        acc[rt] = c;
      }
    };
    auto mfma_tile_l = [&](const u32x4 (&zB)[ND8], f32x16 (&acc)[2]) {
#pragma unroll
      for (int rt = 0; rt < 2; ++rt) {
        f32x16 c = acc[rt];
#pragma unroll
        for (int nb = 0; nb < ND8; ++nb)
          c = __builtin_amdgcn_mfma_f32_32x32x16_bf16(a2v[rt][nb], __builtin_bit_cast(bf16x8, zB[nb]), c, 0, 0, 0);
        acc[rt] = c;
      }
    };
    auto tile_max = [&](const f32x16 (&acc)[2]) {
      float m4[4] = {0.0f, 0.0f, 0.0f, 0.0f};
#pragma unroll
      for (int r = 0; r < 16; ++r)
        m4[r & 3] = fmaxf(fmaxf(m4[r & 3], fabsf(acc[r >> 3][2 * (r & 7)])), fabsf(acc[r >> 3][2 * (r & 7) + 1]));
      return fmaxf(fmaxf(m4[0], m4[1]), fmaxf(m4[2], m4[3]));
    };
    auto reduce_tile = [&](auto collm, const f32x16 (&acc)[2], float mx, float wc) {
      constexpr int CC = decltype(collm)::value;
      f32x2 xx[16];
#pragma unroll
      for (int r = 0; r < 16; ++r) xx[r] = (f32x2){acc[r >> 3][2 * (r & 7)], acc[r >> 3][2 * (r & 7) + 1]};
      f32x2 part2;
      if (CC == 0 && !__any(mx > MM_TIER1_MAX)) {
        if constexpr (ND8 == 1) part2 = mm_weighted_rem1(xx, wc0, wc1);
        else part2 = mm_weighted_rem<1, 0>(xx, wrow);
      } else if (!__any(mx > MM_C6_MAX)) {
        if constexpr (CC == 1) part2 = (f32x2){0.0f, 0.0f};
        else part2 = mm_weighted_rem<3, CC>(xx, wrow);
      } else if (!__any(mx > 0.5f)) {
        part2 = mm_weighted_rem<4, CC>(xx, wrow);
      } else if (!__any(mx > 1.0f)) {
        part2 = mm_weighted_rem<5, CC>(xx, wrow);
      } else {
        part2 = (f32x2){0.0f, 0.0f};
#pragma unroll
        for (int r = 0; r < 16; ++r)
#pragma unroll
          for (int e2 = 0; e2 < 2; ++e2) {
            const float x = fminf(xx[r][e2], MM_EXP_CAP_F32);
            const float xs = fminf(fmaxf(x, -1.0f), 1.0f);
            const float big = (__builtin_amdgcn_exp2f(x * 1.44269504f) - 1.0f) - fmaf(0.5f * x, x, x);
            float e = (fabsf(x) <= 1.0f) ? mm_rem_p5(xs) : big;
            if constexpr (CC == 1) e -= (x * x) * x * fmaf(fmaf(fmaf(MM_C6_C3, x, MM_C6_C2), x, MM_C6_C1), x, MM_C6_C0);
            if constexpr (CC == 2) e -= (x * x) * (x * MM_C6_C0);
            part2[e2] = fmaf(wrow[r >> 3][r & 7][e2], e, part2[e2]);
          }
      }
      sum += (double)wc * (double)(part2[0] + part2[1]);
    };
    auto process_tile = [&](auto collc, auto collm, int ct, const u32x4 (&zA)[ND8], u32x4 (&zB)[ND8], float wc, float& emx, float& ewc) __attribute__((always_inline)) {
      constexpr bool CM = decltype(collc)::value;
      f32x16 acc[2];
      emx = 0.0f; ewc = 0.0f;
      mfma_tile_screen(zA, acc);
      if constexpr (CM) {
        const float ms = tile_max(acc);
        if (!__any(ms > thr_skip)) return;
      }
      mfma_tile_m(zA, acc);
      const float mx = force_worst ? 2.0f : tile_max(acc);
      if constexpr (CM) {
        if (!__any(mx > MM_C6_MAX)) return;
      }
      if constexpr (CM) wc = wcf[ct * 32 + l31];
      emx = mx; ewc = wc;
      if (__any(mx > MM_TWO_WAY_MAX)) {
        if constexpr (CM) load_zB(ct, zB);
        mfma_tile_l(zB, acc);
      }
      reduce_tile(collm, acc, mx, wc);
    };

    int ct_first = 0;
    if (coll) {
      const float a2w = g2 * 1.000001f;
      const float* zt = zt2 + (size_t)a2 * nct;
      int cf = nct;
      for (int c0 = 0; c0 < nct; c0 += 64) {
        const int c = c0 + lane;
        const bool outside = c < nct && a2w * zt[c < nct ? c : 0] > MM_INSIDE_BOUND2;
        const unsigned long long bal = __ballot(outside);
        if (bal) { cf = c0 + (int)__builtin_ctzll(bal); break; }
      }
      ct_first = cf & ~1;
    }
    auto sweep = [&](auto collc, auto collm) __attribute__((always_inline)) {
      constexpr bool CM = decltype(collc)::value;
      u32x4 zA0[ND8], zB0[ND8], zA1[ND8], zB1[ND8];
      float w0, w1;
      w0 = w1 = 0.0f;
      const int ct0 = CM ? ct_first : 0;
      if (ct0 >= nct) return;
      load_zA(ct0, zA0);
      if constexpr (!CM) { load_zB(0, zB0); w0 = wcf[l31]; }
      for (int ct = ct0; ct < nct; ct += 2) {
        load_zA(ct + 1, zA1);
        if constexpr (!CM) { load_zB(ct + 1, zB1); w1 = wcf[(ct + 1) * 32 + l31]; }
        float emx0, ewc0, emx1, ewc1;
        process_tile(collc, collm, ct, zA0, zB0, w0, emx0, ewc0);
        const int cn = ct + 2 < nct ? ct + 2 : ct;
        load_zA(cn, zA0);
        if constexpr (!CM) { load_zB(cn, zB0); w0 = wcf[cn * 32 + l31]; }
        process_tile(collc, collm, ct + 1, zA1, zB1, w1, emx1, ewc1);
#if MM_ROUTE_EST
        {
          const f32x2 emx = {emx0, emx1}, ewc = {ewc0, ewc1};
          const f32x2 u = (emx * emx) * (emx * ewc);
          est2 = mm_pkfma(u, u, est2);
          xall = fmaxf(fmaxf(xall, emx0), emx1);
        }
#endif
      }
    };
    if (coll) sweep(mm_true{}, mm_int<1>{});
    else if (icoll) sweep(mm_false{}, mm_int<2>{});
    else sweep(mm_false{}, mm_int<0>{});
  }
  float estl;
  {
    const float xf = fminf(xall, 8.0f);
    const float pf = fmaxf(fmaf(xf, xf, xf) + 1.0f, __expf(xf));
    estl = ((est2[0] + est2[1]) * rowsq) * (pf * pf);
  }
#pragma unroll
  for (int off = 32; off > 0; off >>= 1) { sum += __shfl_down(sum, off, 64); estl += __shfl_down(estl, off, 64); }
  __syncthreads();
  if (lane == 0) { red[wv] = sum; redf[wv] = estl; }
  __syncthreads();
  if (threadIdx.x == 0) {
    partB[((size_t)b * P + p) * NS + panel] = red[0] + red[1] + red[2] + red[3];
    if (estO) estO[((size_t)b * Po + lp) * npanel + panel] = (redf[0] + redf[1]) + (redf[2] + redf[3]);
  }
  }
}

template <int ND8>
__device__ __forceinline__ void mm_f32_wave_rows(const char* zlds, const float* wlds,
                                                 int row0, int b, int lp, int a2, int Mp, int d, int Po, int force_worst,
                                                 bool icoll, size_t grp0, const unsigned int* __restrict__ amaxc,
                                                 const unsigned char* __restrict__ gflag, const float* __restrict__ gmax2,
                                                 const double* __restrict__ zmax2, const float* __restrict__ zt2,
                                                 const float* __restrict__ rowO,
                                                 double& sum_out, float& estl_out) {
  const int lane = threadIdx.x & 63, l31 = lane & 31, h = lane >> 5;
  double sum = 0.0;
  f32x2 est2 = {0.0f, 0.0f};
  float rowsq = 0.0f, xall = 0.0f;
  const bool coll = icoll && row0 < Mp && gflag[grp0 + (row0 >> 6)] != 0;
  const float g2 = coll ? gmax2[grp0 + (row0 >> 6)] : 0.0f;
  const bool wave_inside = coll && mm_collapse_bound2(__float_as_uint(g2), zmax2[a2]) <= MM_INSIDE_BOUND2;
  if (row0 < Mp && !wave_inside) {
    const float* ra = rowO + ((size_t)b * Po + lp) * (size_t)(d + 1) * Mp;
    const float bound2 = zmax2 ? mm_collapse_bound2(amaxc[(size_t)b * Po + lp], zmax2[a2]) : 3.0e38f;
    const float thr_skip = MM_C6_MAX - 0.00390625f * __builtin_sqrtf(bound2) - 1e-6f;

    bf16x8 a1[2][ND8], a2v[2][ND8], a3[2][ND8];
    f32x2 wrow[2][8], wc0[2][8], wc1[2][8];
#pragma unroll
    for (int rt = 0; rt < 2; ++rt) {
      const int row = row0 + rt * 32 + l31;
#pragma unroll
      for (int nb = 0; nb < ND8; ++nb) {
        unsigned int hh[8], mm[8], ll[8];
#pragma unroll
        for (int j = 0; j < 8; ++j) {
          const int k = nb * 8 + j;
          const float v = ra[(size_t)(k < d ? k : d) * Mp + row];
          mm_split3(k < d ? v : 0.0f, hh[j], mm[j], ll[j]);
        }
        u32x4 ph, pm, pl;
#pragma unroll
        for (int j = 0; j < 4; ++j) {
          ph[j] = hh[2 * j] | (hh[2 * j + 1] << 16);
          pm[j] = mm[2 * j] | (mm[2 * j + 1] << 16);
          pl[j] = ll[2 * j] | (ll[2 * j + 1] << 16);
        }
        a1[rt][nb] = __builtin_bit_cast(bf16x8, pm);
        a2v[rt][nb] = __builtin_bit_cast(bf16x8, h ? pl : ph);
        a3[rt][nb] = __builtin_bit_cast(bf16x8, ph);
      }
#pragma unroll
      for (int g = 0; g < 4; ++g) {
        const int rr = row0 + rt * 32 + 8 * g + 4 * h;
        const float4 v = *reinterpret_cast<const float4*>(ra + (size_t)d * Mp + rr);
        wrow[rt][2 * g + 0] = (f32x2){v.x, v.y};
        wrow[rt][2 * g + 1] = (f32x2){v.z, v.w};
        if constexpr (ND8 == 1) {
#pragma unroll
          for (int q2 = 0; q2 < 2; ++q2) {
            wc0[rt][2 * g + q2] = wrow[rt][2 * g + q2] * MM_PK(MMRem<1>::c[0]);
            wc1[rt][2 * g + q2] = wrow[rt][2 * g + q2] * MM_PK(MMRem<1>::c[1]);
          }
        }
      }
    }
    {
      f32x2 rs = {0.0f, 0.0f};
#pragma unroll
      for (int rt = 0; rt < 2; ++rt)
#pragma unroll
        for (int r = 0; r < 8; ++r) rs = mm_pkfma(wrow[rt][r], wrow[rt][r], rs);
      rowsq = rs[0] + rs[1];
    }

    const unsigned int tile_bytes = 32u * 48u * ND8, part_bytes = 32u * 16u * ND8;
    const unsigned int offA = (h ? 0u : 1u) * part_bytes + (unsigned int)l31 * (16u * ND8);
    const unsigned int offB = (h ? 0u : 2u) * part_bytes + (unsigned int)l31 * (16u * ND8);
    const int nct = Mp >> 5;

    auto load_zA = [&](int ct, u32x4 (&zA)[ND8]) {
#pragma unroll
      for (int nb = 0; nb < ND8; ++nb) zA[nb] = *reinterpret_cast<const u32x4*>(zlds + (size_t)ct * tile_bytes + offA + nb * 16);
    };
    auto load_zB = [&](int ct, u32x4 (&zB)[ND8]) {
#pragma unroll
      for (int nb = 0; nb < ND8; ++nb) zB[nb] = *reinterpret_cast<const u32x4*>(zlds + (size_t)ct * tile_bytes + offB + nb * 16);
    };
    auto load_wc = [&](int j) { return wlds[j]; };

    auto mfma_tile_screen = [&](const u32x4 (&zA)[ND8], f32x16 (&acc)[2]) {
#pragma unroll
      for (int rt = 0; rt < 2; ++rt) {
        f32x16 c = {0.f, 0.f, 0.f, 0.f, 0.f, 0.f, 0.f, 0.f, 0.f, 0.f, 0.f, 0.f, 0.f, 0.f, 0.f, 0.f};
#pragma unroll
        for (int nb = 0; nb < ND8; ++nb)
          c = __builtin_amdgcn_mfma_f32_32x32x16_bf16(a3[rt][nb], __builtin_bit_cast(bf16x8, zA[nb]), c, 0, 0, 0);
        acc[rt] = c;
      }
    };
    auto mfma_tile_m = [&](const u32x4 (&zA)[ND8], f32x16 (&acc)[2]) {
#pragma unroll
      for (int rt = 0; rt < 2; ++rt) {
        f32x16 c = acc[rt];
#pragma unroll
        for (int nb = 0; nb < ND8; ++nb)
          c = __builtin_amdgcn_mfma_f32_32x32x16_bf16(a1[rt][nb], __builtin_bit_cast(bf16x8, zA[nb]), c, 0, 0, 0);
        acc[rt] = c;
      }
    };
    auto mfma_tile_l = [&](const u32x4 (&zB)[ND8], f32x16 (&acc)[2]) {
#pragma unroll
      for (int rt = 0; rt < 2; ++rt) {
        f32x16 c = acc[rt];
#pragma unroll
        for (int nb = 0; nb < ND8; ++nb)
          c = __builtin_amdgcn_mfma_f32_32x32x16_bf16(a2v[rt][nb], __builtin_bit_cast(bf16x8, zB[nb]), c, 0, 0, 0);
        acc[rt] = c;
      }
    };
    auto tile_max = [&](const f32x16 (&acc)[2]) {
      float m4[4] = {0.0f, 0.0f, 0.0f, 0.0f};
#pragma unroll
      for (int r = 0; r < 16; ++r)
        m4[r & 3] = fmaxf(fmaxf(m4[r & 3], fabsf(acc[r >> 3][2 * (r & 7)])), fabsf(acc[r >> 3][2 * (r & 7) + 1]));
      return fmaxf(fmaxf(m4[0], m4[1]), fmaxf(m4[2], m4[3]));
    };
    auto reduce_tile = [&](auto collm, const f32x16 (&acc)[2], float mx, float wc) {
      constexpr int CC = decltype(collm)::value;
      f32x2 xx[16];
#pragma unroll
      for (int r = 0; r < 16; ++r) xx[r] = (f32x2){acc[r >> 3][2 * (r & 7)], acc[r >> 3][2 * (r & 7) + 1]};
      f32x2 part2;
      if (CC == 0 && !__any(mx > MM_TIER1_MAX)) {
        if constexpr (ND8 == 1) part2 = mm_weighted_rem1(xx, wc0, wc1);
        else part2 = mm_weighted_rem<1, 0>(xx, wrow);
      } else if (!__any(mx > MM_C6_MAX)) {
        if constexpr (CC == 1) part2 = (f32x2){0.0f, 0.0f};
        else part2 = mm_weighted_rem<3, CC>(xx, wrow);
      } else if (!__any(mx > 0.5f)) {
        part2 = mm_weighted_rem<4, CC>(xx, wrow);
      } else if (!__any(mx > 1.0f)) {
        part2 = mm_weighted_rem<5, CC>(xx, wrow);
      } else {
        part2 = (f32x2){0.0f, 0.0f};
#pragma unroll
        for (int r = 0; r < 16; ++r)
#pragma unroll
          for (int e2 = 0; e2 < 2; ++e2) {
            const float x = fminf(xx[r][e2], MM_EXP_CAP_F32);
            const float xs = fminf(fmaxf(x, -1.0f), 1.0f);
            const float big = (__builtin_amdgcn_exp2f(x * 1.44269504f) - 1.0f) - fmaf(0.5f * x, x, x);
            float e = (fabsf(x) <= 1.0f) ? mm_rem_p5(xs) : big;
            if constexpr (CC == 1) e -= (x * x) * x * fmaf(fmaf(fmaf(MM_C6_C3, x, MM_C6_C2), x, MM_C6_C1), x, MM_C6_C0);
            if constexpr (CC == 2) e -= (x * x) * (x * MM_C6_C0);
            part2[e2] = fmaf(wrow[r >> 3][r & 7][e2], e, part2[e2]);
          }
      }
      sum += (double)wc * (double)(part2[0] + part2[1]);
    };
    auto process_tile = [&](auto collc, auto collm, int ct, const u32x4 (&zA)[ND8], u32x4 (&zB)[ND8], float wc, float& emx, float& ewc) __attribute__((always_inline)) {
      constexpr bool CM = decltype(collc)::value;
      f32x16 acc[2];
      emx = 0.0f; ewc = 0.0f;
      mfma_tile_screen(zA, acc);
      if constexpr (CM) {
        const float ms = tile_max(acc);
        if (!__any(ms > thr_skip)) return;
      }
      mfma_tile_m(zA, acc);
      const float mx = force_worst ? 2.0f : tile_max(acc);
      if constexpr (CM) {
        if (!__any(mx > MM_C6_MAX)) return;
      }
      if constexpr (CM) wc = load_wc(ct * 32 + l31);
      emx = mx; ewc = wc;
      if (__any(mx > MM_TWO_WAY_MAX)) {
        if constexpr (CM) load_zB(ct, zB);
        mfma_tile_l(zB, acc);
      }
      reduce_tile(collm, acc, mx, wc);
    };

    int ct_first = 0;
    if (coll) {
      const float a2w = g2 * 1.000001f;
      const float* zt = zt2 + (size_t)a2 * nct;
      int cf = nct;
      for (int c0 = 0; c0 < nct; c0 += 64) {
        const int c = c0 + lane;
        const bool outside = c < nct && a2w * zt[c < nct ? c : 0] > MM_INSIDE_BOUND2;
        const unsigned long long bal = __ballot(outside);
        if (bal) { cf = c0 + (int)__builtin_ctzll(bal); break; }
      }
      ct_first = cf & ~1;
    }
    auto sweep = [&](auto collc, auto collm) __attribute__((always_inline)) {
      constexpr bool CM = decltype(collc)::value;
      u32x4 zA0[ND8], zB0[ND8], zA1[ND8], zB1[ND8];
      float w0, w1;
      w0 = w1 = 0.0f;
      const int ct0 = CM ? ct_first : 0;
      if (ct0 >= nct) return;
      load_zA(ct0, zA0);
      if constexpr (!CM) { load_zB(0, zB0); w0 = load_wc(l31); }
      for (int ct = ct0; ct < nct; ct += 2) {
        load_zA(ct + 1, zA1);
        if constexpr (!CM) { load_zB(ct + 1, zB1); w1 = load_wc((ct + 1) * 32 + l31); }
        float emx0, ewc0, emx1, ewc1;
        process_tile(collc, collm, ct, zA0, zB0, w0, emx0, ewc0);
        const int cn = ct + 2 < nct ? ct + 2 : ct;
        load_zA(cn, zA0);
        if constexpr (!CM) { load_zB(cn, zB0); w0 = load_wc(cn * 32 + l31); }
        process_tile(collc, collm, ct + 1, zA1, zB1, w1, emx1, ewc1);
#if MM_ROUTE_EST
        {
          const f32x2 emx = {emx0, emx1}, ewc = {ewc0, ewc1};
          const f32x2 u = (emx * emx) * (emx * ewc);
          est2 = mm_pkfma(u, u, est2);
          xall = fmaxf(fmaxf(xall, emx0), emx1);
        }
#endif
      }
    };
    if (coll) sweep(mm_true{}, mm_int<1>{});
    else if (icoll) sweep(mm_false{}, mm_int<2>{});
    else sweep(mm_false{}, mm_int<0>{});
  }
  {
    const float xf = fminf(xall, 8.0f);
    const float pf = fmaxf(fmaf(xf, xf, xf) + 1.0f, __expf(xf));
    estl_out = ((est2[0] + est2[1]) * rowsq) * (pf * pf);
  }
  sum_out = sum;
}

#ifndef MM_F32P_WAVES
#define MM_F32P_WAVES 8
#endif
#define MM_F32P_MAX_MP 2048
static inline size_t mm_f32p_lds_bytes(int Mp) {
  return (size_t)Mp * 48 + (size_t)Mp * 4 + (size_t)mm_mfma_groups(Mp) * 12;
}

__global__ __launch_bounds__(256) void k_offdiag_worklist(int L, int Mp, int P, int Po, int NS, int npanel, int B, int force_worst,
                                                          const unsigned int* __restrict__ amax, const unsigned int* __restrict__ amaxc,
                                                          const unsigned char* __restrict__ gflag, const float* __restrict__ gmax2,
                                                          const double* __restrict__ zmax2, double* __restrict__ partB,
                                                          float* __restrict__ estO, int* __restrict__ plist, int* __restrict__ rcount) {
  if (blockIdx.x == 0 && threadIdx.x == 0) { rcount[0] = 0; rcount[1] = 0; }
  const int item = blockIdx.x * 4 + (int)(threadIdx.x >> 6), lane = threadIdx.x & 63;
  if (item >= B * Po) return;
  const int b = item / Po, lp = item - b * Po, p = L + lp;
  int a, a2;
  mm_decode_pair_o(p, L, a, a2);
  bool work = true, dense = true;
  if (!force_worst) {
    if (mm_collapse_bound2(amax[item], zmax2[a2]) <= MM_INSIDE_BOUND2) {
      work = false;
    } else if (mm_item_collapsed(amaxc[item])) {
      const int ng = Mp / MM_GROUP_ROWS;
      const size_t grp0 = (size_t)item * ng;
      bool need = false, dn = false;
      for (int g = lane; g < ng; g += 64) {
        const bool coll = gflag[grp0 + g] != 0;
        need = need || !(coll && mm_collapse_bound2(__float_as_uint(gmax2[grp0 + g]), zmax2[a2]) <= MM_INSIDE_BOUND2);
        dn = dn || !coll;
      }
      work = __any(need);
      dense = __any(dn);
    }
  }
  if (!work) {
    for (int panel = lane; panel < npanel; panel += 64) {
      partB[((size_t)b * P + p) * NS + panel] = 0.0;
      estO[(size_t)item * npanel + panel] = 0.0f;
    }
    return;
  }
  if (lane == 0) {
    int* list = plist + mm_f32p_list_off(L);
    const int off = B * (a2 * (a2 - 1) / 2), cap = B * a2;
    if (dense) list[off + atomicAdd(plist + 4 + 2 * a2, 1)] = item;
    else list[off + cap - 1 - atomicAdd(plist + 5 + 2 * a2, 1)] = item;
  }
}

__global__ __launch_bounds__(64 * MM_F32P_WAVES, 1) void k_qred_f32_mfma_persist(const unsigned short* __restrict__ Zs3, int L, int Mp,
                                                                               int d, int P, int Po, int NS, int npanel, int B,
                                                                               int force_worst, const unsigned int* __restrict__ amaxc,
                                                                               const unsigned char* __restrict__ gflag,
                                                                               const float* __restrict__ gmax2,
                                                                               const double* __restrict__ zmax2,
                                                                               const float* __restrict__ zt2,
                                                                               const float* __restrict__ rowO,
                                                                               const float* __restrict__ colO,
                                                                               double* __restrict__ partB, float* __restrict__ estO,
                                                                               int* __restrict__ plist) {
  constexpr int NT = 64 * MM_F32P_WAVES;
  extern __shared__ __align__(16) char zlds[];
  __shared__ int s_next, s_gcur;
  const int tid = threadIdx.x, lane = tid & 63;
  const int ngrp = mm_mfma_groups(Mp);
  float* wlds = reinterpret_cast<float*>(zlds + (size_t)Mp * 48);
  double* red = reinterpret_cast<double*>(wlds + Mp);
  float* redf = reinterpret_cast<float*>(red + ngrp);
  const int* cnt = plist + 4;
  const int* list = plist + mm_f32p_list_off(L);
  int total = 0;
  for (int c = 1; c < L; ++c) total += cnt[2 * c] + cnt[2 * c + 1];
  if (tid == 0) s_next = atomicAdd(plist, 1);
  __syncthreads();
  int cur = -1;
  for (;;) {
    int r = __builtin_amdgcn_readfirstlane(s_next);
    if (r >= total) break;
    int c = 1;
    while (r >= cnt[2 * c] + cnt[2 * c + 1]) { r -= cnt[2 * c] + cnt[2 * c + 1]; ++c; }
    const int boff = B * (c * (c - 1) / 2);
    const int item = __builtin_amdgcn_readfirstlane(list[boff + (r < cnt[2 * c] ? r : B * c - 1 - (r - cnt[2 * c]))]);
    const int b = item / Po, lp = item - b * Po, p = L + lp;
    int a, a2;
    mm_decode_pair_o(p, L, a, a2);
    int ft = tid;
    asm volatile("" : "+v"(ft));
    if (a2 != cur) {
      const char* src = reinterpret_cast<const char*>(Zs3 + (size_t)a2 * Mp * 24);
      const int nchunk = Mp * 3;
      for (int c0 = 0; c0 < nchunk; c0 += 8 * NT) {
        u32x4 tmp[8];
#pragma unroll
        for (int u = 0; u < 8; ++u) {
          const int ch = c0 + u * NT + ft;
          tmp[u] = *reinterpret_cast<const u32x4*>(src + (size_t)(ch < nchunk ? ch : nchunk - 1) * 16);
        }
#pragma unroll
        for (int u = 0; u < 8; ++u) {
          const int ch = c0 + u * NT + ft;
          if (ch < nchunk) *reinterpret_cast<u32x4*>(zlds + (size_t)ch * 16) = tmp[u];
        }
      }
      cur = a2;
    }
    {
      const float* src = colO + (size_t)item * Mp;
      for (int ch = ft; ch < Mp / 4; ch += NT)
        reinterpret_cast<u32x4*>(wlds)[ch] = *reinterpret_cast<const u32x4*>(src + (size_t)ch * 4);
    }
    if (tid == 0) s_gcur = 0;
    __syncthreads();
    if (tid == 0) s_next = atomicAdd(plist, 1);
    const bool icoll = !force_worst && mm_item_collapsed(amaxc[item]);
    const size_t grp0 = (size_t)item * (size_t)(Mp / MM_GROUP_ROWS);
    for (int gi = __builtin_amdgcn_readfirstlane(atomicAdd(&s_gcur, lane == 0 ? 1 : 0)); gi < ngrp;
         gi = __builtin_amdgcn_readfirstlane(atomicAdd(&s_gcur, lane == 0 ? 1 : 0))) {
      const int g = ngrp - 1 - gi;
      double sum;
      float estl;
      mm_f32_wave_rows<1>(zlds, wlds, g * 64, b, lp, a2, Mp, d, Po, force_worst, icoll, grp0, amaxc, gflag, gmax2, zmax2, zt2, rowO,
                          sum, estl);
#pragma unroll
      for (int off = 32; off > 0; off >>= 1) { sum += __shfl_down(sum, off, 64); estl += __shfl_down(estl, off, 64); }
      if (lane == 0) { red[g] = sum; redf[g] = estl; }
    }
    __syncthreads();
    for (int panel = tid; panel < npanel; panel += NT) {
      const double* rp = red + 4 * panel;
      const float* rf = redf + 4 * panel;
      partB[((size_t)b * P + p) * NS + panel] = rp[0] + rp[1] + rp[2] + rp[3];
      estO[(size_t)item * npanel + panel] = (rf[0] + rf[1]) + (rf[2] + rf[3]);
    }
  }
}

extern "C" int mm_mfma_supported(int d) { return d >= 1 && d <= 32; }

int mm_mfma_num_slots(int Mp) { return (Mp + MM_PANEL_ROWS - 1) / MM_PANEL_ROWS; }

int mm_launch_qred_mfma(const char* packed, const MMModelLayout& ml, char* ws, const MMWorkspaceLayout& wl,
                        int B, int L, int d, int flags, hipStream_t stream) {
  const int npanel = mm_mfma_num_slots(wl.Mp);
  const int force_worst = (flags & MM_FORCE_WORST_TIER) ? 1 : 0;
  const unsigned int* amax = (const unsigned int*)(ws + wl.amax);
  const double* zmax2 = mm_moment_deg(d) >= 4 ? (const double*)(packed + ml.zmax2) : nullptr;
  const size_t zbytes = (size_t)wl.Mp * 32 * ml.nd8;
  const bool ldsz = ml.nd8 == 1 && zbytes <= 65536;
  int ppw = 1;
  if (ldsz && (long long)wl.Po * B >= 4096) ppw = (npanel + MM_F32_PPW_DIV - 1) / MM_F32_PPW_DIV;
  const long long nwork_ll = (long long)((npanel + ppw - 1) / ppw) * wl.Po * B;
  if (nwork_ll <= 0 || nwork_ll > 0x7fffffffLL) return MM_E_DIM;
  const int nwork = (int)nwork_ll;
  const unsigned short* Zs3 = (const unsigned short*)(packed + ml.Zs3);
  const float* rowO = (const float*)(ws + wl.rowO);
  const float* colO = (const float*)(ws + wl.colO);
  double* partB = (double*)(ws + wl.partB);
  float* estO = (float*)(ws + wl.estO);
  if (ml.nd8 == 1 && zmax2 && wl.Mp <= MM_F32P_MAX_MP && !force_worst && !(flags & MM_ISTAGE_OLD_OFFDIAG)) {
    int* plist = (int*)(ws + wl.plist);
    const int nitem = wl.Po * B;
    const hipError_t em = hipMemsetAsync(plist, 0, (size_t)mm_f32p_list_off(L) * 4, stream);
    if (em != hipSuccess) return (int)em;
    hipLaunchKernelGGL(k_offdiag_worklist, dim3((nitem + 3) / 4), dim3(256), 0, stream, L, wl.Mp, wl.P, wl.Po, wl.NS, npanel, B,
                       force_worst, amax, (const unsigned int*)(ws + wl.amaxc), (const unsigned char*)(ws + wl.gflag),
                       (const float*)(ws + wl.gmax2), zmax2, partB, estO, plist, (int*)(ws + wl.rcount));
    const hipError_t el = hipGetLastError();
    if (el != hipSuccess) return (int)el;
    const size_t shm = mm_f32p_lds_bytes(wl.Mp);
    static std::atomic<unsigned long long> attr_done{0ull};
    static std::atomic<int> ncu_cached[64];
    int dev = 0;
    if (hipGetDevice(&dev) != hipSuccess) dev = 64;
    const unsigned long long bit = (dev >= 0 && dev < 64) ? (1ull << dev) : 0ull;
    int ncu = bit ? ncu_cached[dev].load() : 0;
    if (!bit || !(attr_done.load() & bit)) {
      const hipError_t ea = hipFuncSetAttribute((const void*)k_qred_f32_mfma_persist, hipFuncAttributeMaxDynamicSharedMemorySize,
                                                (int)mm_f32p_lds_bytes(MM_F32P_MAX_MP));
      if (ea != hipSuccess) return (int)ea;
      int v = 0;
      if (hipDeviceGetAttribute(&v, hipDeviceAttributeMultiprocessorCount, dev < 64 ? dev : 0) != hipSuccess || v <= 0) v = 256;
      ncu = v;
      if (bit) { ncu_cached[dev].store(v); attr_done.fetch_or(bit); }
    }
    if (ncu <= 0) ncu = 256;
    hipLaunchKernelGGL(k_qred_f32_mfma_persist, dim3(nitem < ncu ? nitem : ncu), dim3(64 * MM_F32P_WAVES), shm, stream, Zs3, L, wl.Mp,
                       d, wl.P, wl.Po, wl.NS, npanel, B, force_worst, (const unsigned int*)(ws + wl.amaxc),
                       (const unsigned char*)(ws + wl.gflag), (const float*)(ws + wl.gmax2), zmax2, (const float*)(packed + ml.zt2),
                       rowO, colO, partB, estO, plist);
    const hipError_t ep = hipGetLastError();
    return ep == hipSuccess ? 0 : (int)ep;
  }
#define MM_LAUNCH_ND(ND_, LZ_, SH_)                                                                          \
  hipLaunchKernelGGL((k_qred_f32_mfma<ND_, LZ_>), dim3(nwork), dim3(256), SH_, stream, Zs3, L, wl.Mp, d,    \
                     wl.P, wl.Po, wl.NS, npanel, ppw, nwork, force_worst, amax, (const unsigned int*)(ws + wl.amaxc), \
                     (const unsigned char*)(ws + wl.gflag), (const float*)(ws + wl.gmax2), zmax2, (const float*)(packed + ml.zt2), rowO, colO, partB, estO, (int*)(ws + wl.rcount))
  switch (ml.nd8) {
    case 1: if (ldsz) MM_LAUNCH_ND(1, true, zbytes); else MM_LAUNCH_ND(1, false, 0); break;
    case 2: MM_LAUNCH_ND(2, false, 0); break;
    case 3: MM_LAUNCH_ND(3, false, 0); break;
    default: MM_LAUNCH_ND(4, false, 0); break;
  }
#undef MM_LAUNCH_ND
  hipError_t e = hipGetLastError();
  return e == hipSuccess ? 0 : (int)e;
}
```

gpflowpilco_amd/ops.py:

```python
from __future__ import annotations

from dataclasses import dataclass, field
from typing import Dict, Optional, Tuple

import torch

from . import _lib
from ._lib import (MM_F32, MM_F64, MM_FORCE_GENERIC, MM_FULL_OUTPUT_COV, MM_WORKSPACE_CURRENT, MM_SUMS_CURRENT,
                   MM_MODEL_UNCERTAINTY, check, lib)

_DTYPES = {torch.float32: MM_F32, torch.float64: MM_F64}


def _dtype_code(dtype: torch.dtype) -> int:
  try:
    return _DTYPES[dtype]
  except KeyError:
    raise TypeError(f"moment matching supports float32/float64 states, got {dtype}") from None


def _ptr(t: Optional[torch.Tensor]):
  return None if t is None else t.data_ptr()


# ... 122 lines not shown
  if mu.dtype != pm.dtype or Sigma.dtype != pm.dtype:
    raise TypeError(f"state dtype {mu.dtype}/{Sigma.dtype} does not match the packed model ({pm.dtype})")
  B, d = mu.shape
  if d != pm.d or Sigma.shape != (B, d, d):
    raise ValueError(f"expected mu [B,{pm.d}] and Sigma [B,{pm.d},{pm.d}], got {tuple(mu.shape)}, {tuple(Sigma.shape)}")
  return B, mu.contiguous(), Sigma.contiguous()


def moment_match(pm: PackedModel, mu: torch.Tensor, Sigma: torch.Tensor,
                 full_output_cov: bool = True, model_uncertainty: bool = True,
                 jitter: float = 0.0, force_generic: bool = False, extra_flags: int = 0):
  B, mu, Sigma = _prep_state(pm, mu, Sigma)
  flags = make_flags(full_output_cov, model_uncertainty, force_generic) | int(extra_flags)
  f1 = torch.empty(B, pm.L, dtype=pm.dtype, device=pm.device)
  Sff = torch.empty((B, pm.L, pm.L) if full_output_cov else (B, pm.L), dtype=pm.dtype, device=pm.device)
  cross = torch.empty(B, pm.d, pm.L, dtype=pm.dtype, device=pm.device)
  if B == 0:
    if model_uncertainty and not pm.with_C:
      check(-5, "mm_moment_match")
    return f1, Sff, cross
  ws = pm.workspace(B, flags)
  rc = lib().mm_moment_match(pm.buf.data_ptr(), pm.nbytes, pm.L, pm.M, pm.d, _dtype_code(pm.dtype), B,
                             mu.data_ptr(), Sigma.data_ptr(), flags, float(jitter),
                             f1.data_ptr(), Sff.data_ptr(), cross.data_ptr(),
                             ws.data_ptr(), ws.numel(), pm.status().data_ptr(), _stream(pm.device))
  check(rc, "mm_moment_match")
  return f1, Sff, cross


def q_forward(pm: PackedModel, mu: torch.Tensor, Sigma: torch.Tensor, flags: int, want_q: bool = False):
  B, mu, Sigma = _prep_state(pm, mu, Sigma)
  ws = pm.workspace(B, flags)
  f1 = torch.empty(B, pm.L, dtype=pm.dtype, device=pm.device)
  cross = torch.empty(B, pm.d, pm.L, dtype=pm.dtype, device=pm.device)
  q = torch.empty(B, pm.L, pm.M, dtype=pm.dtype, device=pm.device) if want_q else None
  rc = lib().mm_q_forward(pm.buf.data_ptr(), pm.nbytes, pm.L, pm.M, pm.d, _dtype_code(pm.dtype), B,
                          mu.data_ptr(), Sigma.data_ptr(), flags, f1.data_ptr(), cross.data_ptr(), _ptr(q),
                          ws.data_ptr(), ws.numel(), pm.status().data_ptr(), _stream(pm.device))
  check(rc, "mm_q_forward")
  return f1, cross, q


def Q_reduce_forward(pm: PackedModel, B: int, flags: int, jitter: float = 0.0):
  ws = pm.workspace(B, flags)
  full = bool(flags & MM_FULL_OUTPUT_COV)
  Sff = torch.empty((B, pm.L, pm.L) if full else (B, pm.L), dtype=pm.dtype, device=pm.device)
  rc = lib().mm_Q_reduce_forward(pm.buf.data_ptr(), pm.nbytes, pm.L, pm.M, pm.d, _dtype_code(pm.dtype), B,
                                 flags, float(jitter), Sff.data_ptr(), ws.data_ptr(), ws.numel(),
                                 _stream(pm.device))
  check(rc, "mm_Q_reduce_forward")
  return Sff


def offdiag_stats(pm: PackedModel, B: int, flags: int):
  ws = pm.workspace(B, flags, peek=True)
  out = torch.zeros(6, dtype=torch.int32, device=pm.device)
  rc = lib().mm_offdiag_stats(pm.buf.data_ptr(), pm.nbytes, pm.L, pm.M, pm.d, _dtype_code(pm.dtype), B, flags,
                              ws.data_ptr(), ws.numel(), out.data_ptr(), _stream(pm.device))
  check(rc, "mm_offdiag_stats")
  c, n, inside, _, _, _ = out.tolist()
  return c, n, inside


def offdiag_row_groups(pm: PackedModel, B: int, flags: int):
  ws = pm.workspace(B, flags, peek=True)
  out = torch.zeros(6, dtype=torch.int32, device=pm.device)
  rc = lib().mm_offdiag_stats(pm.buf.data_ptr(), pm.nbytes, pm.L, pm.M, pm.d, _dtype_code(pm.dtype), B, flags,
                              ws.data_ptr(), ws.numel(), out.data_ptr(), _stream(pm.device))
  check(rc, "mm_offdiag_stats")
  o = out.tolist()
  Mp = (pm.M + _lib.MM_M_ALIGN - 1) // _lib.MM_M_ALIGN * _lib.MM_M_ALIGN
  return o[4], o[5], o[1] * (Mp // 64)


def offdiag_routed(pm: PackedModel, B: int, flags: int) -> int:
  if pm.dtype != torch.float32 or pm.L < 2 or not (flags & MM_FULL_OUTPUT_COV):
    return 0
  ws = pm.workspace(B, flags, peek=True)
  out = torch.zeros(6, dtype=torch.int32, device=pm.device)
  rc = lib().mm_offdiag_stats(pm.buf.data_ptr(), pm.nbytes, pm.L, pm.M, pm.d, _dtype_code(pm.dtype), B, flags,
                              ws.data_ptr(), ws.numel(), out.data_ptr(), _stream(pm.device))
  check(rc, "mm_offdiag_stats")
  return int(out[3])


def route_estimates(pm: PackedModel, B: int, flags: int) -> torch.Tensor:
  Po = pm.L * (pm.L - 1) // 2 if (flags & MM_FULL_OUTPUT_COV) else 0
  out = torch.zeros(B, Po, 2, dtype=torch.float64, device=pm.device)
  if Po:
    ws = pm.workspace(B, flags, peek=True)
    rc = lib().mm_route_estimates(pm.buf.data_ptr(), pm.nbytes, pm.L, pm.M, pm.d, _dtype_code(pm.dtype), B, flags,
                                  ws.data_ptr(), ws.numel(), out.data_ptr(), _stream(pm.device))
    check(rc, "mm_route_estimates")
  return out


def euler_update(mu, Sigma, f1, Sff, cross_pre, dt: float = 1.0):
  _require_device(mu, Sigma, f1, Sff, cross_pre)
  B, d = mu.shape
  if f1.shape != (B, d) or Sff.shape != (B, d, d) or cross_pre.shape != (B, d, d):
    raise ValueError("euler_update needs d == L and a full output covariance")
  args = [t.contiguous() for t in (mu, Sigma, f1, Sff, cross_pre)]
  mu_o, S_o = torch.empty_like(args[0]), torch.empty_like(args[1])
  rc = lib().mm_euler_update(B, d, _dtype_code(mu.dtype), float(dt), *[t.data_ptr() for t in args],
                             mu_o.data_ptr(), S_o.data_ptr(), _stream(mu.device))
  check(rc, "mm_euler_update")
  return mu_o, S_o


def rollout_closed(pm: PackedModel, mu: torch.Tensor, Sigma: torch.Tensor, num_steps: int,
                   dt: float = 1.0, model_uncertainty: bool = True, jitter: float = 0.0,
                   keep_trajectory: bool = False, force_generic: bool = False):
  B, mu, Sigma = _prep_state(pm, mu, Sigma)
  mu, Sigma = mu.clone(), Sigma.clone()
  flags = make_flags(True, model_uncertainty, force_generic)
  ws = pm.workspace(B, flags)
  tmu = tS = None
  if keep_trajectory:
    tmu = torch.empty(num_steps, B, pm.d, dtype=pm.dtype, device=pm.device)
    tS = torch.empty(num_steps, B, pm.d, pm.d, dtype=pm.dtype, device=pm.device)
  rc = lib().mm_rollout_closed(pm.buf.data_ptr(), pm.nbytes, pm.L, pm.M, pm.d, _dtype_code(pm.dtype), B,
                               int(num_steps), float(dt), flags, float(jitter),
                               mu.data_ptr(), Sigma.data_ptr(), _ptr(tmu), _ptr(tS),
                               ws.data_ptr(), ws.numel(), pm.status().data_ptr(), _stream(pm.device))
  check(rc, "mm_rollout_closed")
  return (mu, Sigma, tmu, tS) if keep_trajectory else (mu, Sigma)


class GraphedRollout:

  def __init__(self, pm: PackedModel, B: int, num_steps: int, dt: float = 1.0, model_uncertainty: bool = True,
               jitter: float = 0.0, keep_trajectory: bool = False):
    if pm.L != pm.d:
      raise ValueError("closed rollout needs state dim == d == L")
    self.pm, self.B, self.H = pm, int(B), int(num_steps)
    kw = dict(dtype=pm.dtype, device=pm.device)
    self.mu_in, self.S_in = torch.zeros(B, pm.d, **kw), torch.eye(pm.d, **kw).expand(B, pm.d, pm.d).contiguous()
    self.mu, self.S = torch.empty(B, pm.d, **kw), torch.empty(B, pm.d, pm.d, **kw)
    self.tmu = torch.empty(num_steps, B, pm.d, **kw) if keep_trajectory else None
    self.tS = torch.empty(num_steps, B, pm.d, pm.d, **kw) if keep_trajectory else None
    flags = make_flags(True, model_uncertainty, False)
    self._flags = flags
    ws = pm.workspace(B, flags)
    status = pm.status()

    def enqueue():
      self.mu.copy_(self.mu_in); self.S.copy_(self.S_in)
      rc = lib().mm_rollout_closed(pm.buf.data_ptr(), pm.nbytes, pm.L, pm.M, pm.d, _dtype_code(pm.dtype), self.B,
                                   self.H, float(dt), flags, float(jitter),
                                   self.mu.data_ptr(), self.S.data_ptr(), _ptr(self.tmu), _ptr(self.tS),
                                   ws.data_ptr(), ws.numel(), status.data_ptr(), _stream(pm.device))
      check(rc, "mm_rollout_closed")

    side = torch.cuda.Stream(device=pm.device)
    side.wait_stream(torch.cuda.current_stream(pm.device))
    with torch.cuda.stream(side):
      enqueue()
    torch.cuda.current_stream(pm.device).wait_stream(side)
    torch.cuda.synchronize(pm.device)
    status.zero_()
    self.graph = torch.cuda.CUDAGraph()
    with torch.cuda.graph(self.graph):
      enqueue()

  def __call__(self, mu: torch.Tensor, Sigma: torch.Tensor):
    if tuple(mu.shape) != (self.B, self.pm.d) or tuple(Sigma.shape) != (self.B, self.pm.d, self.pm.d):
# ... 462 lines not shown
```

include/gpflowpilco_mm.h:

```cpp
#ifndef GPFLOWPILCO_MM_H
#define GPFLOWPILCO_MM_H

#include <stddef.h>
#include <stdint.h>

#ifdef __cplusplus
extern "C" {
#endif

#define MM_F32 0
#define MM_F64 1

#define MM_DMAX 32
#define MM_M_ALIGN 128

#define MM_FULL_OUTPUT_COV   1
#define MM_MODEL_UNCERTAINTY 2
#define MM_FORCE_GENERIC     4
#define MM_STAGE_DIAG        8
#define MM_STAGE_OFFDIAG    16
#define MM_STAGE_FINALIZE   32
#define MM_FORCE_WORST_TIER 64
#define MM_WORKSPACE_CURRENT 128
#define MM_FORCE_ROUTE 256
#define MM_NO_ROUTE 512
#define MM_SUMS_CURRENT 1024

#define MM_E_ARG      (-1)
#define MM_E_DIM      (-2)
#define MM_E_DTYPE    (-3)
#define MM_E_WORKSPACE (-4)
#define MM_E_NO_C     (-5)
#define MM_E_STATE    (-6)

int mm_abi_version(void);

size_t mm_packed_model_bytes(int L, int M, int d, int dtype, int with_C);

int mm_pack_model(void* packed, size_t packed_bytes,
                  int L, int M, int d, int dtype,
                  const double* Z,
                  const double* lengthscales,
                  const double* variance,
                  const double* beta,
                  const double* C,
                  const double* mean_c,
                  void* stream);

int mm_pack_perm(const void* packed, size_t packed_bytes, int L, int M, int d, int dtype, int32_t* perm, void* stream);

size_t mm_workspace_bytes(int B, int L, int M, int d, int dtype, int flags);

int mm_moment_match(const void* packed, size_t packed_bytes, int L, int M, int d, int dtype,
                    int B,
                    const void* mu,
                    const void* Sigma,
                    int flags, double jitter,
                    void* f1,
                    void* Sff,
                    void* cross_pre,
                    void* workspace, size_t workspace_bytes,
                    int32_t* status, void* stream);

int mm_q_forward(const void* packed, size_t packed_bytes, int L, int M, int d, int dtype, int B,
                 const void* mu, const void* Sigma, int flags,
                 void* f1, void* cross_pre, void* q_out,
                 void* workspace, size_t workspace_bytes, int32_t* status, void* stream);

int mm_Q_reduce_forward(const void* packed, size_t packed_bytes, int L, int M, int d, int dtype, int B,
                        int flags, double jitter, void* Sff,
                        void* workspace, size_t workspace_bytes, void* stream);

int mm_euler_update(int B, int d, int dtype, double dt,
                    const void* mu, const void* Sigma,
                    const void* f1, const void* Sff, const void* cross_pre,
                    void* mu_out, void* Sigma_out, void* stream);

int mm_rollout_closed(const void* packed, size_t packed_bytes, int L, int M, int d, int dtype, int B, int H,
                      double dt, int flags, double jitter,
                      void* mu, void* Sigma, void* traj_mu, void* traj_Sigma,
                      void* workspace, size_t workspace_bytes,
                      int32_t* status, void* stream);

int mm_expected_cost(int N, int d, int dtype, const void* mean, const void* cov,
                     const void* target, const void* precis, void* cost, void* stream);

int mm_offdiag_stats(const void* packed, size_t packed_bytes, int L, int M, int d, int dtype, int B, int flags,
                     const void* workspace, size_t workspace_bytes, int32_t* out, void* stream);

int mm_route_estimates(const void* packed, size_t packed_bytes, int L, int M, int d, int dtype, int B, int flags,
                       const void* workspace, size_t workspace_bytes, double* out, void* stream);

size_t mm_compose_workspace_bytes(int B, int nx, int na, int dtype);
int mm_rollout_composed(const void* drift_packed, size_t drift_bytes, int drift_L, int drift_M, int drift_d,
                        const void* policy_packed, size_t policy_bytes, int policy_M, int policy_d,
                        int dtype, int B, int H, double dt, int nx, int na, const int32_t* active_dims,
                        double head_scale, double head_shift, const void* target, const void* precis,
                        void* mx, void* Sxx, void* cost, void* traj_mu, void* traj_Sigma,
                        void* ws_drift, size_t ws_drift_bytes, void* ws_policy, size_t ws_policy_bytes,
                        void* ws_compose, size_t ws_compose_bytes, int32_t* status, void* stream);

size_t mm_compose_nd_workspace_bytes(int B, int nx, int na, int nu, int dtype);
int mm_rollout_composed_nd(const void* drift_packed, size_t drift_bytes, int drift_L, int drift_M, int drift_d,
                           const void* policy_packed, size_t policy_bytes, int policy_M, int policy_d,
                           int dtype, int B, int H, double dt, int nx, int na, const int32_t* active_dims,
                           int nu, const double* head_scale, const double* head_shift,
                           const void* target, const void* precis,
                           void* mx, void* Sxx, void* cost, void* traj_mu, void* traj_Sigma,
                           void* ws_drift, size_t ws_drift_bytes, void* ws_policy, size_t ws_policy_bytes,
                           void* ws_compose, size_t ws_compose_bytes, int32_t* status, void* stream);

size_t mm_compose_tape_bytes(int B, int H, int nx, int na, int drift_M, int dtype);
int mm_rollout_composed_taped(const void* drift_packed, size_t drift_bytes, int drift_L, int drift_M, int drift_d,
                              const void* policy_packed, size_t policy_bytes, int policy_M, int policy_d,
                              int dtype, int B, int H, double dt, int nx, int na, const int32_t* active_dims,
                              double head_scale, double head_shift, const void* target, const void* precis,
                              void* mx, void* Sxx, void* cost, void* ws_drift, size_t ws_drift_bytes,
                              void* ws_policy, size_t ws_policy_bytes, void* tape, size_t tape_bytes,
                              int32_t* status, void* stream);

size_t mm_compose_backward_workspace_bytes(int B, int nx, int na, int drift_M);
size_t mm_policy_grad_bytes(int B, int policy_M, int policy_d);
int mm_rollout_composed_backward(const void* drift_packed, size_t drift_bytes, int drift_L, int drift_M, int drift_d,
                                 const void* policy_packed, size_t policy_bytes, int policy_M, int policy_d,
                                 int dtype, int B, int H, double dt, int nx, int na, const int32_t* active_dims,
                                 double head_scale, double head_shift, const void* target, const void* precis,
                                 const void* tape, size_t tape_bytes, const void* g_cost,
                                 void* g_policy, void* g_mx0, void* g_Sxx0,
                                 void* ws_drift, size_t ws_drift_bytes, void* ws_bwd, size_t ws_bwd_bytes,
                                 int32_t* status, void* stream);

int mm_rollout_composed_backward_seeded(const void* drift_packed, size_t drift_bytes, int drift_L, int drift_M, int drift_d,
                                        const void* policy_packed, size_t policy_bytes, int policy_M, int policy_d,
                                        int dtype, int B, int H, double dt, int nx, int na, const int32_t* active_dims,
                                        double head_scale, double head_shift, const void* target, const void* precis,
                                        const void* tape, size_t tape_bytes, const void* g_cost,
                                        const void* g_xm, const void* g_xS,
                                        void* g_policy, void* g_mx0, void* g_Sxx0,
                                        void* ws_drift, size_t ws_drift_bytes, void* ws_bwd, size_t ws_bwd_bytes,
                                        int32_t* status, void* stream);

size_t mm_compose_tape_bytes_nd(int B, int H, int nx, int na, int nu, int drift_M, int dtype);
int mm_rollout_composed_taped_nd(const void* drift_packed, size_t drift_bytes, int drift_L, int drift_M, int drift_d,
                                 const void* policy_packed, size_t policy_bytes, int policy_M, int policy_d,
                                 int dtype, int B, int H, double dt, int nx, int na, const int32_t* active_dims,
                                 int nu, const double* head_scale, const double* head_shift,
                                 const void* target, const void* precis, void* mx, void* Sxx, void* cost,
                                 void* ws_drift, size_t ws_drift_bytes, void* ws_policy, size_t ws_policy_bytes,
                                 void* tape, size_t tape_bytes, int32_t* status, void* stream);
size_t mm_compose_backward_workspace_bytes_nd(int B, int nx, int na, int nu, int drift_M, int policy_M);
size_t mm_policy_grad_bytes_nd(int B, int nu, int policy_M, int policy_d);
int mm_rollout_composed_backward_nd(const void* drift_packed, size_t drift_bytes, int drift_L, int drift_M, int drift_d,
                                    const void* policy_packed, size_t policy_bytes, int policy_M, int policy_d,
                                    int dtype, int B, int H, double dt, int nx, int na, const int32_t* active_dims,
                                    int nu, const double* head_scale, const double* head_shift,
                                    const void* target, const void* precis, const void* tape, size_t tape_bytes,
                                    const void* g_cost, void* g_policy, void* g_mx0, void* g_Sxx0,
                                    void* ws_drift, size_t ws_drift_bytes, void* ws_bwd, size_t ws_bwd_bytes,
                                    int32_t* status, void* stream);
int mm_rollout_composed_backward_nd_seeded(const void* drift_packed, size_t drift_bytes, int drift_L, int drift_M, int drift_d,
                                           const void* policy_packed, size_t policy_bytes, int policy_M, int policy_d,
                                           int dtype, int B, int H, double dt, int nx, int na, const int32_t* active_dims,
                                           int nu, const double* head_scale, const double* head_shift,
                                           const void* target, const void* precis, const void* tape, size_t tape_bytes,
                                           const void* g_cost, const void* g_xm, const void* g_xS,
                                           void* g_policy, void* g_mx0, void* g_Sxx0,
                                           void* ws_drift, size_t ws_drift_bytes, void* ws_bwd, size_t ws_bwd_bytes,
                                           int32_t* status, void* stream);

size_t mm_compose_nd_mixed_workspace_bytes(int B, int nx, int na, int nu, int drift_L, int dtype);
int mm_rollout_composed_nd_mixed(const void* drift_packed, size_t drift_bytes, int drift_L, int drift_M, int drift_d,
// ... 194 lines not shown
```

Measured before the change: 43530 rollout step-elements/s (B*H per rollout second).

## Tighten off-diagonal skip bounds with lengthscale-scaled norms and column tile ranges

Adds lengthscale-scaled per-tile inducing-point norms (zt2s) and per-group scaled row bounds (gmax2s), and uses their product as a tighter test for whether a tile lies inside the collapse bound in the f32 MFMA off-diagonal Q reduction. The column sweep now also stops at the last outside tile, not only starting at the first, so more tiles and whole work items can be skipped. This adds extra bound computation and storage in the pairvec kernel, a wave reduction in the worklist kernel, and debug entry points and flags. The risk is that the scaled bound is only valid if the product inequality truly bounds the exponent, and if not, required contributions could be dropped.

```diff
diff --git a/gpflowpilco_amd/_lib.py b/gpflowpilco_amd/_lib.py
--- a/gpflowpilco_amd/_lib.py
+++ b/gpflowpilco_amd/_lib.py
@@ -20,6 +20,8 @@
 MM_FORCE_ROUTE = 256
 MM_NO_ROUTE = 512
 MM_SUMS_CURRENT = 1024
+MM_ISTAGE_OLD_SKIP_BOUND = 1 << 26
+MM_ISTAGE_NO_BOUND_SKIP = 1 << 27
 
 ERRORS = {
     -1: "MM_E_ARG: NULL pointer or non-positive size",
@@ -52,6 +54,9 @@
     "mm_expected_cost": (C.c_int, [C.c_int, C.c_int, C.c_int] + [C.c_void_p] * 6),
     "mm_offdiag_stats": (C.c_int, [C.c_void_p, C.c_size_t, C.c_int, C.c_int, C.c_int, C.c_int, C.c_int, C.c_int,
                                    C.c_void_p, C.c_size_t, C.c_void_p, C.c_void_p]),
+    "mm_offdiag_worklist_len": (C.c_int, [C.c_int] * 6 + [C.c_void_p, C.c_size_t, C.c_void_p, C.c_void_p]),
+    "mm_offdiag_skip_bounds": (C.c_int, [C.c_void_p, C.c_size_t, C.c_int, C.c_int, C.c_int, C.c_int, C.c_int, C.c_int,
+                                         C.c_void_p, C.c_size_t, C.c_void_p, C.c_void_p, C.c_void_p]),
     "mm_route_estimates": (C.c_int, [C.c_void_p, C.c_size_t, C.c_int, C.c_int, C.c_int, C.c_int, C.c_int, C.c_int,
                                      C.c_void_p, C.c_size_t, C.c_void_p, C.c_void_p]),
     "mm_compose_workspace_bytes": (C.c_size_t, [C.c_int] * 4),
diff --git a/gpflowpilco_amd/csrc/mm_common.h b/gpflowpilco_amd/csrc/mm_common.h
--- a/gpflowpilco_amd/csrc/mm_common.h
+++ b/gpflowpilco_amd/csrc/mm_common.h
@@ -13,6 +13,8 @@
 #define MM_ISTAGE_OLD_OFFDIAG (1 << 23)
 #define MM_ISTAGE_OLD_SPOLY56 (1 << 24)
 #define MM_ISTAGE_OLD_DIAG_MAP (1 << 25)
+#define MM_ISTAGE_OLD_SKIP_BOUND (1 << 26)
+#define MM_ISTAGE_NO_BOUND_SKIP (1 << 27)
 
 #define MM_PW_KERNELS 3
 
@@ -72,6 +74,7 @@
   size_t perm;
   size_t skey;
   size_t zt2;
+  size_t zt2s;
   size_t Cm;
   size_t total;
 };
@@ -110,6 +113,7 @@
   o.perm = off;   off = mm_align_up(off + (size_t)L * o.Mp * 4, A);
   o.skey = off;   off = mm_align_up(off + (size_t)L * o.Mp * 8, A);
   o.zt2 = off;    off = mm_align_up(off + (size_t)L * (o.Mp / 32) * 4, A);
+  o.zt2s = off;   off = mm_align_up(off + (size_t)L * (o.Mp / 32) * 4, A);
   o.Cm = off;
   if (with_C) off = mm_align_up(off + (size_t)L * o.Mp * o.Mp * 8, A);
   o.total = off;
@@ -191,6 +195,7 @@
   size_t gperm;
   size_t s12;
   size_t gmax2;
+  size_t gmax2s;
   size_t partB;
   size_t partC;
   size_t mu64;
@@ -247,6 +252,7 @@
   o.amaxc = off;   off = mm_align_up(off + (size_t)B * o.Po * 4, A);
   o.gflag = off;   off = mm_align_up(off + (dtype == MM_F64 ? 0 : (size_t)B * o.Po * (o.Mp / 64)), A);
   o.gmax2 = off;   off = mm_align_up(off + (dtype == MM_F64 ? 0 : (size_t)B * o.Po * (o.Mp / 64) * 4), A);
+  o.gmax2s = off;  off = mm_align_up(off + (dtype == MM_F64 ? 0 : (size_t)B * o.Po * (o.Mp / 64) * 4), A);
   o.gperm = off;   off = mm_align_up(off + (dtype == MM_F64 || L < 2 ? 0 : ((size_t)L * (L - 1) * B + 3 * L) * 4), A);
   o.s12 = off;     off = mm_align_up(off + (size_t)B * o.Po * 8, A);
   o.partB = off;   off = mm_align_up(off + (size_t)B * o.P * o.NS * 8, A);
diff --git a/gpflowpilco_amd/csrc/mm_kernels.hip b/gpflowpilco_amd/csrc/mm_kernels.hip
--- a/gpflowpilco_amd/csrc/mm_kernels.hip
+++ b/gpflowpilco_amd/csrc/mm_kernels.hip
@@ -213,16 +213,23 @@
     if (tid == 0) ((double*)(packed + lay.zmax2))[a] = fmax(fmax(red[0], red[1]), fmax(red[2], red[3]));
     __syncthreads();
     float* zt2 = (float*)(packed + lay.zt2) + (size_t)a * (lay.Mp / 32);
+    float* zt2s = (float*)(packed + lay.zt2s) + (size_t)a * (lay.Mp / 32);
     for (int t = tid; t < lay.Mp / 32; t += 256) {
-      double mx = 0.0;
+      double mx = 0.0, mxs = 0.0;
       for (int j = 0; j < 32; ++j) {
         const int m = t * 32 + j;
         if (m >= M) break;
-        double s2 = 0.0;
-        for (int k = 0; k < d; ++k) { const double v = Z[((size_t)a * M + m) * d + k] - zb[k]; s2 += v * v; }
+        double s2 = 0.0, s2s = 0.0;
+        for (int k = 0; k < d; ++k) {
+          const double v = Z[((size_t)a * M + m) * d + k] - zb[k], l = ls[a * d + k];
+          s2 += v * v;
+          s2s += v * v / (l * l);
+        }
         mx = s2 > mx ? s2 : mx;
+        mxs = s2s > mxs ? s2s : mxs;
       }
       zt2[t] = (float)(mx * 1.000001);
+      zt2s[t] = (float)(mxs * 1.000001);
     }
   }
   if (sizeof(T) != 8) {
@@ -568,7 +575,8 @@
                                                  double* __restrict__ qhC, int with_unc, int nblk,
                                                  const double* __restrict__ lq, const double* __restrict__ beta64,
                                                  const double* __restrict__ zmax2, unsigned short* __restrict__ ,
-                                                 unsigned char* __restrict__ , float* __restrict__ , int , int p0) {
+                                                 unsigned char* __restrict__ , float* __restrict__ , float* __restrict__ ,
+                                                 int , int p0) {
   static_assert(DK > 8, "d <= 8 takes k_pairvec_reg");
   const int p = p0 + (int)blockIdx.y, b = blockIdx.z, tid = threadIdx.x;
   int a, a2;
@@ -716,7 +724,7 @@
                                                     double (*vecs)[DK], const double* __restrict__ lq,
                                                     const double* __restrict__ beta64, int p, const double* __restrict__ zmax2,
                                                     unsigned short* __restrict__ wsp, unsigned char* __restrict__ gflag, float* __restrict__ gmax2,
-                                                    int allow) {
+                                                    float* __restrict__ gmax2s, int allow) {
   constexpr bool diag = MODE == 0;
   const int b = blockIdx.z, tid = threadIdx.x;
   const int Po = P - L;
@@ -817,6 +825,7 @@
   const double cst = pm[d * d];
   float a2max = 0.0f;
   float a2cmax = 0.0f, a2in = 0.0f;
+  float a2sin = 0.0f;
   const bool cancoll = MODE == 1 && allow && recentred;
   const double zm2c = MODE == 1 ? zmax2[a2] : 0.0;
   typedef const __attribute__((address_space(3))) double* lds_cptr;
@@ -876,7 +885,7 @@
           sr[k] = (o.zr[k] - muk) * vl[DK + k]; sc[k] = (o.zc[k] - muk) * vl[2 * DK + k];
           cj = fma(vl[5 * DK + k], sc[k], cj);
         }
-        double tA = 0.0, tg = 0.0, corrA = 0.0, asq = 0.0;
+        double tA = 0.0, tg = 0.0, corrA = 0.0, asq = 0.0, asqs = 0.0;
 #pragma unroll
         for (int i = 0; i < DK; ++i) {
           double u = 0.0, vh = 0.0;
@@ -890,6 +899,7 @@
           tg = fma(sc[i], fma(2.0, vh, Tr[tsym(i, i)] * sc[i]), tg);
           const double av = (u + vl[5 * DK + i]) * vl[2 * DK + i];
           asq = fma(av, av, asq);
+          asqs = fma(u + vl[5 * DK + i], av, asqs);
           corrA = fma(vl[3 * DK + i], u, corrA);
           rO[rowi(i) + m] = (T)av;
         }
@@ -897,12 +907,13 @@
         a2max = fmaxf(a2max, a2row);
         rowok = mm_collapse_bound2(__float_as_uint(a2row), zm2c) <= MM_COLLAPSE_BOUND2;
         a2in = a2row;
+        a2sin = (float)asqs * 1.000001f;
         whr = o.br * exp(fmin(o.wr - 0.5 * (o.r1r - tA) + cst - corrA, (double)MM_EXP_CAP_F32));
         whc = o.bc * exp(fmin(o.wc - 0.5 * (o.r1c - tg) - cj, (double)MM_EXP_CAP_F32));
       } else {
 #pragma unroll
         for (int i = 0; i < DK; ++i) rO[rowi(i) + m] = (T)0;
-        a2in = 0.0f;
+        a2in = 0.0f; a2sin = 0.0f;
       }
       rO[rowd + m] = (T)whr; cO[m] = (T)whc; hR[m] = whr; hC[m] = whc;
       if (wsp) {
@@ -910,10 +921,14 @@
         float g2 = a2in;
 #pragma unroll
         for (int off = 32; off > 0; off >>= 1) g2 = fmaxf(g2, __shfl_xor(g2, off, 64));
+        float g2s = a2sin;
+#pragma unroll
+        for (int off = 32; off > 0; off >>= 1) g2s = fmaxf(g2s, __shfl_xor(g2s, off, 64));
         if ((tid & 63) == 0) {
           const size_t gi = ((size_t)b * Po + (p - L)) * (size_t)(Mp / MM_GROUP_ROWS) + (m >> 6);
           gflag[gi] = inner ? 1 : 0;
           gmax2[gi] = g2;
+          gmax2s[gi] = g2s;
         }
         if (inner) a2cmax = fmaxf(a2cmax, a2in);
         unsigned short* sp = wsp + ((size_t)b * Po + (p - L)) * 4 * (size_t)Mp + m;
@@ -986,7 +1001,8 @@
                                                         double* __restrict__ qhC, int with_unc, int nblk,
                                                         const double* __restrict__ lq, const double* __restrict__ beta64,
                                                         const double* __restrict__ zmax2, unsigned short* __restrict__ wsp,
-                                                        unsigned char* __restrict__ gflag, float* __restrict__ gmax2, int allow, int p0) {
+                                                        unsigned char* __restrict__ gflag, float* __restrict__ gmax2,
+                                                        float* __restrict__ gmax2s, int allow, int p0) {
   static_assert(DK <= 8, "register form: d <= 8");
   __shared__ double vecs[7][DK];
   const int p = p0 + (int)blockIdx.y;
@@ -994,7 +1010,7 @@
   mm_decode_pair(p, L, a, a2);
 #define MM_PV_BODY(MODE_)                                                                                           \
   mm_pairvec_reg_body<T, DK, MODE_>(Zt64, zbar, ls2, L, M, Mp, d, P, mu, pairmat, rho1, rowD, colD, rowO, colO, w64, \
-                                    whR, whC, amax, q64, qhR, qhC, with_unc, nblk, a, a2, vecs, lq, beta64, p, zmax2, wsp, gflag, gmax2, allow)
+                                    whR, whC, amax, q64, qhR, qhC, with_unc, nblk, a, a2, vecs, lq, beta64, p, zmax2, wsp, gflag, gmax2, gmax2s, allow)
   if (p < L) MM_PV_BODY(0);
   else if (sizeof(T) == 4) MM_PV_BODY(1);
   else MM_PV_BODY(2);
@@ -1286,7 +1302,7 @@
     (const double*)(ws + wl.q64), (double*)(ws + wl.qhR), (double*)(ws + wl.qhC), (flags & MM_MODEL_UNCERTAINTY) ? 1 : 0, nblk, \
     (const double*)(ws + wl.lq), (const double*)(packed + ml.beta64), (const double*)(packed + ml.zmax2),                       \
     ((sizeof(T) == 4 && d <= 8) ? (unsigned short*)(ws + wl.wsp) : (unsigned short*)nullptr),                                \
-    (unsigned char*)(ws + wl.gflag), (float*)(ws + wl.gmax2), ((flags & (MM_FORCE_WORST_TIER | MM_ISTAGE_NO_M56)) ? 0 : 1)
+    (unsigned char*)(ws + wl.gflag), (float*)(ws + wl.gmax2), (float*)(ws + wl.gmax2s), ((flags & (MM_FORCE_WORST_TIER | MM_ISTAGE_NO_M56)) ? 0 : 1)
     auto pairvec = [&](int p0, int npairs, hipStream_t st) {
       if (npairs <= 0) return;
       if constexpr (DK <= 8) {
diff --git a/gpflowpilco_amd/csrc/mm_mfma.hip b/gpflowpilco_amd/csrc/mm_mfma.hip
--- a/gpflowpilco_amd/csrc/mm_mfma.hip
+++ b/gpflowpilco_amd/csrc/mm_mfma.hip
@@ -9,6 +9,19 @@
   int r = p - L, i = 0;
   while (r >= L - 1 - i) { r -= L - 1 - i; ++i; }
   a = i; a2 = i + 1 + r;
+}
+
+__device__ __forceinline__ float mm_wave_max_tiles(const float* __restrict__ zt, int nct, int lane) {
+  float m = 0.0f;
+  for (int c = lane; c < nct; c += 64) m = fmaxf(m, zt[c]);
+#pragma unroll
+  for (int off = 32; off > 0; off >>= 1) m = fmaxf(m, __shfl_xor(m, off, 64));
+  return m;
+}
+__device__ __forceinline__ bool mm_group_inside(const float* __restrict__ gmax2, const float* __restrict__ gmax2s, size_t gi,
+                                                double zmax2a, float zsmax) {
+  return gmax2s ? (gmax2s[gi] * 1.000001f) * zsmax <= MM_INSIDE_BOUND2
+                : mm_collapse_bound2(__float_as_uint(gmax2[gi]), zmax2a) <= MM_INSIDE_BOUND2;
 }
 
 #ifndef MM_TWO_WAY_MAX
@@ -80,6 +93,8 @@
                                                           const unsigned int* __restrict__ amaxc,
                                                           const unsigned char* __restrict__ gflag, const float* __restrict__ gmax2,
                                                           const double* __restrict__ zmax2, const float* __restrict__ zt2,
+                                                          const float* __restrict__ gmax2s, const float* __restrict__ zt2s,
+                                                          int noskip,
                                                           const float* __restrict__ rowO,
                                                           const float* __restrict__ colO,
                                                           double* __restrict__ partB, float* __restrict__ estO,
@@ -99,7 +114,8 @@
 
   const int wv = threadIdx.x >> 6, lane = threadIdx.x & 63, l31 = lane & 31, h = lane >> 5;
   if constexpr (ND8 == 1) {
-    if (!force_worst && zmax2 && mm_collapse_bound2(amax[(size_t)b * Po + lp], zmax2[a2]) <= MM_INSIDE_BOUND2) {
+    if (!force_worst && zmax2 && mm_collapse_bound2(amax[(size_t)b * Po + lp], zmax2[a2]) <= MM_INSIDE_BOUND2 &&
+        !(noskip && mm_item_collapsed(amaxc[(size_t)b * Po + lp]))) {
       for (int panel = (int)threadIdx.x; panel < npanel; panel += 256) {
         if (panel % npw != pgrp) continue;
         partB[((size_t)b * P + p) * NS + panel] = 0.0;
@@ -111,13 +127,15 @@
   const bool icoll_wg = (ND8 == 1) && !force_worst && zmax2 != nullptr && zt2 != nullptr && gmax2 != nullptr &&
                         mm_item_collapsed(amaxc[(size_t)b * Po + lp]);
   const size_t grp0 = ((size_t)b * Po + lp) * (size_t)(Mp / MM_GROUP_ROWS);
+  const bool scaled = gmax2s != nullptr && zt2s != nullptr;
   if constexpr (ND8 == 1) {
-    if (icoll_wg) {
+    if (icoll_wg && !noskip) {
+      const float zsmax = scaled ? mm_wave_max_tiles(zt2s + (size_t)a2 * (Mp >> 5), Mp >> 5, lane) : 0.0f;
       bool need = false;
       for (int panel = pgrp; panel < npanel; panel += npw) {
         const int g = (panel * MM_PANEL_ROWS + wv * 64) >> 6;
         if (g < Mp / MM_GROUP_ROWS)
-          need = need || !(gflag[grp0 + g] != 0 && mm_collapse_bound2(__float_as_uint(gmax2[grp0 + g]), zmax2[a2]) <= MM_INSIDE_BOUND2);
+          need = need || !(gflag[grp0 + g] != 0 && mm_group_inside(gmax2, scaled ? gmax2s : nullptr, grp0 + g, zmax2[a2], zsmax));
       }
       if (!__syncthreads_or(need ? 1 : 0)) {
         for (int panel = (int)threadIdx.x; panel < npanel; panel += 256) {
@@ -159,8 +177,27 @@
   float rowsq = 0.0f, xall = 0.0f;
   const bool icoll = icoll_wg;
   const bool coll = icoll && row0 < Mp && gflag[grp0 + (row0 >> 6)] != 0;
-  const float g2 = coll ? gmax2[grp0 + (row0 >> 6)] : 0.0f;
-  const bool wave_inside = coll && mm_collapse_bound2(__float_as_uint(g2), zmax2[a2]) <= MM_INSIDE_BOUND2;
+  const float g2 = coll ? (scaled ? gmax2s : gmax2)[grp0 + (row0 >> 6)] : 0.0f;
+  int ct_first = 0, ct_end = Mp >> 5;
+  bool wave_inside = false;
+  if (coll && !noskip) {
+    const int nctw = Mp >> 5;
+    const float a2w = g2 * 1.000001f;
+    const float* zt = (scaled ? zt2s : zt2) + (size_t)a2 * nctw;
+    int cf = nctw, cl = -1;
+    for (int c0 = 0; c0 < nctw; c0 += 64) {
+      const int c = c0 + lane;
+      const bool outside = c < nctw && a2w * zt[c < nctw ? c : 0] > MM_INSIDE_BOUND2;
+      const unsigned long long bal = __ballot(outside);
+      if (bal) {
+        if (cf == nctw) cf = c0 + (int)__builtin_ctzll(bal);
+        cl = c0 + 63 - (int)__builtin_clzll(bal);
+      }
+    }
+    ct_first = cf & ~1;
+    if (scaled) ct_end = (cl + 2) & ~1;
+    wave_inside = scaled ? cf >= nctw : mm_collapse_bound2(__float_as_uint(g2), zmax2[a2]) <= MM_INSIDE_BOUND2;
+  }
   if (row0 < Mp && !wave_inside) {
     const float* ra = rowO + ((size_t)b * Po + lp) * (size_t)(d + 1) * Mp;
     const float* wcf = colO + ((size_t)b * Po + lp) * Mp;
@@ -328,34 +365,21 @@
       reduce_tile(collm, acc, mx, wc);
     };
 
-    int ct_first = 0;
-    if (coll) {
-      const float a2w = g2 * 1.000001f;
-      const float* zt = zt2 + (size_t)a2 * nct;
-      int cf = nct;
-      for (int c0 = 0; c0 < nct; c0 += 64) {
-        const int c = c0 + lane;
-        const bool outside = c < nct && a2w * zt[c < nct ? c : 0] > MM_INSIDE_BOUND2;
-        const unsigned long long bal = __ballot(outside);
-        if (bal) { cf = c0 + (int)__builtin_ctzll(bal); break; }
-      }
-      ct_first = cf & ~1;
-    }
     auto sweep = [&](auto collc, auto collm) __attribute__((always_inline)) {
       constexpr bool CM = decltype(collc)::value;
       u32x4 zA0[ND8], zB0[ND8], zA1[ND8], zB1[ND8];
       float w0, w1;
       w0 = w1 = 0.0f;
-      const int ct0 = CM ? ct_first : 0;
-      if (ct0 >= nct) return;
+      const int ct0 = CM ? ct_first : 0, cte = CM ? ct_end : nct;
+      if (ct0 >= cte) return;
       load_zA(ct0, zA0);
       if constexpr (!CM) { load_zB(0, zB0); w0 = wcf[l31]; }
-      for (int ct = ct0; ct < nct; ct += 2) {
+      for (int ct = ct0; ct < cte; ct += 2) {
         load_zA(ct + 1, zA1);
         if constexpr (!CM) { load_zB(ct + 1, zB1); w1 = wcf[(ct + 1) * 32 + l31]; }
         float emx0, ewc0, emx1, ewc1;
         process_tile(collc, collm, ct, zA0, zB0, w0, emx0, ewc0);
-        const int cn = ct + 2 < nct ? ct + 2 : ct;
+        const int cn = ct + 2 < cte ? ct + 2 : ct;
         load_zA(cn, zA0);
         if constexpr (!CM) { load_zB(cn, zB0); w0 = wcf[cn * 32 + l31]; }
         process_tile(collc, collm, ct + 1, zA1, zB1, w1, emx1, ewc1);
@@ -397,15 +421,36 @@
                                                  bool icoll, size_t grp0, const unsigned int* __restrict__ amaxc,
                                                  const unsigned char* __restrict__ gflag, const float* __restrict__ gmax2,
                                                  const double* __restrict__ zmax2, const float* __restrict__ zt2,
+                                                 const float* __restrict__ gmax2s, const float* __restrict__ zt2s, int noskip,
                                                  const float* __restrict__ rowO,
                                                  double& sum_out, float& estl_out) {
   const int lane = threadIdx.x & 63, l31 = lane & 31, h = lane >> 5;
+  const bool scaled = gmax2s != nullptr && zt2s != nullptr;
   double sum = 0.0;
   f32x2 est2 = {0.0f, 0.0f};
   float rowsq = 0.0f, xall = 0.0f;
   const bool coll = icoll && row0 < Mp && gflag[grp0 + (row0 >> 6)] != 0;
-  const float g2 = coll ? gmax2[grp0 + (row0 >> 6)] : 0.0f;
-  const bool wave_inside = coll && mm_collapse_bound2(__float_as_uint(g2), zmax2[a2]) <= MM_INSIDE_BOUND2;
+  const float g2 = coll ? (scaled ? gmax2s : gmax2)[grp0 + (row0 >> 6)] : 0.0f;
+  int ct_first = 0, ct_end = Mp >> 5;
+  bool wave_inside = false;
+  if (coll && !noskip) {
+    const int nctw = Mp >> 5;
+    const float a2w = g2 * 1.000001f;
+    const float* zt = (scaled ? zt2s : zt2) + (size_t)a2 * nctw;
+    int cf = nctw, cl = -1;
+    for (int c0 = 0; c0 < nctw; c0 += 64) {
+      const int c = c0 + lane;
+      const bool outside = c < nctw && a2w * zt[c < nctw ? c : 0] > MM_INSIDE_BOUND2;
+      const unsigned long long bal = __ballot(outside);
+      if (bal) {
+        if (cf == nctw) cf = c0 + (int)__builtin_ctzll(bal);
+        cl = c0 + 63 - (int)__builtin_clzll(bal);
+      }
+    }
+    ct_first = cf & ~1;
+    if (scaled) ct_end = (cl + 2) & ~1;
+    wave_inside = scaled ? cf >= nctw : mm_collapse_bound2(__float_as_uint(g2), zmax2[a2]) <= MM_INSIDE_BOUND2;
+  }
   if (row0 < Mp && !wave_inside) {
     const float* ra = rowO + ((size_t)b * Po + lp) * (size_t)(d + 1) * Mp;
     const float bound2 = zmax2 ? mm_collapse_bound2(amaxc[(size_t)b * Po + lp], zmax2[a2]) : 3.0e38f;
@@ -568,34 +613,21 @@
       reduce_tile(collm, acc, mx, wc);
     };
 
-    int ct_first = 0;
-    if (coll) {
-      const float a2w = g2 * 1.000001f;
-      const float* zt = zt2 + (size_t)a2 * nct;
-      int cf = nct;
-      for (int c0 = 0; c0 < nct; c0 += 64) {
-        const int c = c0 + lane;
-        const bool outside = c < nct && a2w * zt[c < nct ? c : 0] > MM_INSIDE_BOUND2;
-        const unsigned long long bal = __ballot(outside);
-        if (bal) { cf = c0 + (int)__builtin_ctzll(bal); break; }
-      }
-      ct_first = cf & ~1;
-    }
     auto sweep = [&](auto collc, auto collm) __attribute__((always_inline)) {
       constexpr bool CM = decltype(collc)::value;
       u32x4 zA0[ND8], zB0[ND8], zA1[ND8], zB1[ND8];
       float w0, w1;
       w0 = w1 = 0.0f;
-      const int ct0 = CM ? ct_first : 0;
-      if (ct0 >= nct) return;
+      const int ct0 = CM ? ct_first : 0, cte = CM ? ct_end : nct;
+      if (ct0 >= cte) return;
       load_zA(ct0, zA0);
       if constexpr (!CM) { load_zB(0, zB0); w0 = load_wc(l31); }
-      for (int ct = ct0; ct < nct; ct += 2) {
+      for (int ct = ct0; ct < cte; ct += 2) {
         load_zA(ct + 1, zA1);
         if constexpr (!CM) { load_zB(ct + 1, zB1); w1 = load_wc((ct + 1) * 32 + l31); }
         float emx0, ewc0, emx1, ewc1;
         process_tile(collc, collm, ct, zA0, zB0, w0, emx0, ewc0);
-        const int cn = ct + 2 < nct ? ct + 2 : ct;
+        const int cn = ct + 2 < cte ? ct + 2 : ct;
         load_zA(cn, zA0);
         if constexpr (!CM) { load_zB(cn, zB0); w0 = load_wc(cn * 32 + l31); }
         process_tile(collc, collm, ct + 1, zA1, zB1, w1, emx1, ewc1);
@@ -632,7 +664,8 @@
 __global__ __launch_bounds__(256) void k_offdiag_worklist(int L, int Mp, int P, int Po, int NS, int npanel, int B, int force_worst,
                                                           const unsigned int* __restrict__ amax, const unsigned int* __restrict__ amaxc,
                                                           const unsigned char* __restrict__ gflag, const float* __restrict__ gmax2,
-                                                          const double* __restrict__ zmax2, double* __restrict__ partB,
+                                                          const double* __restrict__ zmax2, const float* __restrict__ gmax2s,
+                                                          const float* __restrict__ zt2s, int noskip, double* __restrict__ partB,
                                                           float* __restrict__ estO, int* __restrict__ plist, int* __restrict__ rcount) {
   if (blockIdx.x == 0 && threadIdx.x == 0) { rcount[0] = 0; rcount[1] = 0; }
   const int item = blockIdx.x * 4 + (int)(threadIdx.x >> 6), lane = threadIdx.x & 63;
@@ -642,15 +675,18 @@
   mm_decode_pair_o(p, L, a, a2);
   bool work = true, dense = true;
   if (!force_worst) {
-    if (mm_collapse_bound2(amax[item], zmax2[a2]) <= MM_INSIDE_BOUND2) {
+    const bool ic = mm_item_collapsed(amaxc[item]);
+    if (mm_collapse_bound2(amax[item], zmax2[a2]) <= MM_INSIDE_BOUND2 && !(noskip && ic)) {
       work = false;
-    } else if (mm_item_collapsed(amaxc[item])) {
+    } else if (ic) {
       const int ng = Mp / MM_GROUP_ROWS;
       const size_t grp0 = (size_t)item * ng;
+      const bool scaled = gmax2s != nullptr && zt2s != nullptr;
+      const float zsmax = (scaled && !noskip) ? mm_wave_max_tiles(zt2s + (size_t)a2 * (Mp >> 5), Mp >> 5, lane) : 0.0f;
       bool need = false, dn = false;
       for (int g = lane; g < ng; g += 64) {
         const bool coll = gflag[grp0 + g] != 0;
-        need = need || !(coll && mm_collapse_bound2(__float_as_uint(gmax2[grp0 + g]), zmax2[a2]) <= MM_INSIDE_BOUND2);
+        need = need || noskip || !(coll && mm_group_inside(gmax2, scaled ? gmax2s : nullptr, grp0 + g, zmax2[a2], zsmax));
         dn = dn || !coll;
       }
       work = __any(need);
@@ -679,6 +715,8 @@
                                                                                const float* __restrict__ gmax2,
                                                                                const double* __restrict__ zmax2,
                                                                                const float* __restrict__ zt2,
+                                                                               const float* __restrict__ gmax2s,
+                                                                               const float* __restrict__ zt2s, int noskip,
                                                                                const float* __restrict__ rowO,
                                                                                const float* __restrict__ colO,
                                                                                double* __restrict__ partB, float* __restrict__ estO,
@@ -743,8 +781,8 @@
       const int g = ngrp - 1 - gi;
       double sum;
       float estl;
-      mm_f32_wave_rows<1>(zlds, wlds, g * 64, b, lp, a2, Mp, d, Po, force_worst, icoll, grp0, amaxc, gflag, gmax2, zmax2, zt2, rowO,
-                          sum, estl);
+      mm_f32_wave_rows<1>(zlds, wlds, g * 64, b, lp, a2, Mp, d, Po, force_worst, icoll, grp0, amaxc, gflag, gmax2, zmax2, zt2, gmax2s,
+                          zt2s, noskip, rowO, sum, estl);
 #pragma unroll
       for (int off = 32; off > 0; off >>= 1) { sum += __shfl_down(sum, off, 64); estl += __shfl_down(estl, off, 64); }
       if (lane == 0) { red[g] = sum; redf[g] = estl; }
@@ -761,6 +799,41 @@
 
 extern "C" int mm_mfma_supported(int d) { return d >= 1 && d <= 32; }
 
+__global__ void k_worklist_len(const int* __restrict__ plist, int L, int32_t* __restrict__ out) {
+  int n = 0;
+  for (int c = 1; c < L; ++c) n += plist[4 + 2 * c] + plist[5 + 2 * c];
+  out[0] = n;
+}
+
+extern "C" int mm_offdiag_worklist_len(int L, int M, int d, int dtype, int B, int flags, const void* workspace, size_t workspace_bytes,
+                                       int32_t* out, void* stream) {
+  if (!workspace || !out || L <= 0 || M <= 0 || d <= 0 || d > MM_DMAX || B <= 0) return MM_E_ARG;
+  const MMWorkspaceLayout wl = mm_workspace_layout(B, L, M, d, dtype, flags);
+  if (workspace_bytes < wl.total) return MM_E_WORKSPACE;
+  hipStream_t s = (hipStream_t)stream;
+  const hipError_t e = hipMemsetAsync(out, 0, sizeof(int32_t), s);
+  if (e != hipSuccess) return (int)e;
+  if (dtype != MM_F32 || wl.Po == 0 || d > 8 || wl.Mp > MM_F32P_MAX_MP) return 0;
+  hipLaunchKernelGGL(k_worklist_len, dim3(1), dim3(1), 0, s, (const int*)((const char*)workspace + wl.plist), L, out);
+  const hipError_t el = hipGetLastError();
+  return el == hipSuccess ? 0 : (int)el;
+}
+
+extern "C" int mm_offdiag_skip_bounds(const void* packed, size_t packed_bytes, int L, int M, int d, int dtype, int B, int flags,
+                                      const void* workspace, size_t workspace_bytes, float* zt2s_out, float* gmax2s_out, void* stream) {
+  if (!packed || !workspace || !zt2s_out || !gmax2s_out || L <= 0 || M <= 0 || d <= 0 || d > MM_DMAX || B <= 0) return MM_E_ARG;
+  if (dtype != MM_F32 || d > 8) return MM_E_DIM;
+  const MMModelLayout ml = mm_model_layout(L, M, d, dtype, 1);
+  const MMWorkspaceLayout wl = mm_workspace_layout(B, L, M, d, dtype, flags);
+  if (packed_bytes < ml.Cm || workspace_bytes < wl.total) return MM_E_WORKSPACE;
+  hipStream_t s = (hipStream_t)stream;
+  hipError_t e = hipMemcpyAsync(zt2s_out, (const char*)packed + ml.zt2s, (size_t)L * (ml.Mp / 32) * 4, hipMemcpyDeviceToDevice, s);
+  if (e == hipSuccess && wl.Po > 0)
+    e = hipMemcpyAsync(gmax2s_out, (const char*)workspace + wl.gmax2s, (size_t)B * wl.Po * (wl.Mp / MM_GROUP_ROWS) * 4,
+                       hipMemcpyDeviceToDevice, s);
+  return e == hipSuccess ? 0 : (int)e;
+}
+
 int mm_mfma_num_slots(int Mp) { return (Mp + MM_PANEL_ROWS - 1) / MM_PANEL_ROWS; }
 
 int mm_launch_qred_mfma(const char* packed, const MMModelLayout& ml, char* ws, const MMWorkspaceLayout& wl,
@@ -769,6 +842,10 @@
   const int force_worst = (flags & MM_FORCE_WORST_TIER) ? 1 : 0;
   const unsigned int* amax = (const unsigned int*)(ws + wl.amax);
   const double* zmax2 = mm_moment_deg(d) >= 4 ? (const double*)(packed + ml.zmax2) : nullptr;
+  const bool scaled = zmax2 != nullptr && ml.nd8 == 1 && !(flags & MM_ISTAGE_OLD_SKIP_BOUND);
+  const float* gmax2s = scaled ? (const float*)(ws + wl.gmax2s) : nullptr;
+  const float* zt2s = scaled ? (const float*)(packed + ml.zt2s) : nullptr;
+  const int noskip = (flags & MM_ISTAGE_NO_BOUND_SKIP) ? 1 : 0;
   const size_t zbytes = (size_t)wl.Mp * 32 * ml.nd8;
   const bool ldsz = ml.nd8 == 1 && zbytes <= 65536;
   int ppw = 1;
@@ -788,7 +865,7 @@
     if (em != hipSuccess) return (int)em;
     hipLaunchKernelGGL(k_offdiag_worklist, dim3((nitem + 3) / 4), dim3(256), 0, stream, L, wl.Mp, wl.P, wl.Po, wl.NS, npanel, B,
                        force_worst, amax, (const unsigned int*)(ws + wl.amaxc), (const unsigned char*)(ws + wl.gflag),
-                       (const float*)(ws + wl.gmax2), zmax2, partB, estO, plist, (int*)(ws + wl.rcount));
+                       (const float*)(ws + wl.gmax2), zmax2, gmax2s, zt2s, noskip, partB, estO, plist, (int*)(ws + wl.rcount));
     const hipError_t el = hipGetLastError();
     if (el != hipSuccess) return (int)el;
     const size_t shm = mm_f32p_lds_bytes(wl.Mp);
@@ -811,14 +888,14 @@
     hipLaunchKernelGGL(k_qred_f32_mfma_persist, dim3(nitem < ncu ? nitem : ncu), dim3(64 * MM_F32P_WAVES), shm, stream, Zs3, L, wl.Mp,
                        d, wl.P, wl.Po, wl.NS, npanel, B, force_worst, (const unsigned int*)(ws + wl.amaxc),
                        (const unsigned char*)(ws + wl.gflag), (const float*)(ws + wl.gmax2), zmax2, (const float*)(packed + ml.zt2),
-                       rowO, colO, partB, estO, plist);
+                       gmax2s, zt2s, noskip, rowO, colO, partB, estO, plist);
     const hipError_t ep = hipGetLastError();
     return ep == hipSuccess ? 0 : (int)ep;
   }
 #define MM_LAUNCH_ND(ND_, LZ_, SH_)                                                                          \
   hipLaunchKernelGGL((k_qred_f32_mfma<ND_, LZ_>), dim3(nwork), dim3(256), SH_, stream, Zs3, L, wl.Mp, d,    \
                      wl.P, wl.Po, wl.NS, npanel, ppw, nwork, force_worst, amax, (const unsigned int*)(ws + wl.amaxc), \
-                     (const unsigned char*)(ws + wl.gflag), (const float*)(ws + wl.gmax2), zmax2, (const float*)(packed + ml.zt2), rowO, colO, partB, estO, (int*)(ws + wl.rcount))
+                     (const unsigned char*)(ws + wl.gflag), (const float*)(ws + wl.gmax2), zmax2, (const float*)(packed + ml.zt2), gmax2s, zt2s, noskip, rowO, colO, partB, estO, (int*)(ws + wl.rcount))
   switch (ml.nd8) {
     case 1: if (ldsz) MM_LAUNCH_ND(1, true, zbytes); else MM_LAUNCH_ND(1, false, 0); break;
     case 2: MM_LAUNCH_ND(2, false, 0); break;
diff --git a/gpflowpilco_amd/ops.py b/gpflowpilco_amd/ops.py
--- a/gpflowpilco_amd/ops.py
+++ b/gpflowpilco_amd/ops.py
@@ -228,6 +228,29 @@
                               ws.data_ptr(), ws.numel(), out.data_ptr(), _stream(pm.device))
   check(rc, "mm_offdiag_stats")
   return int(out[3])
+
+
+def offdiag_worklist_len(pm: PackedModel, B: int, flags: int) -> int:
+  if pm.dtype != torch.float32 or pm.L < 2 or not (flags & MM_FULL_OUTPUT_COV):
+    return 0
+  ws = pm.workspace(B, flags, peek=True)
+  out = torch.zeros(1, dtype=torch.int32, device=pm.device)
+  rc = lib().mm_offdiag_worklist_len(pm.L, pm.M, pm.d, _dtype_code(pm.dtype), B, flags, ws.data_ptr(), ws.numel(),
+                                     out.data_ptr(), _stream(pm.device))
+  check(rc, "mm_offdiag_worklist_len")
+  return int(out[0])
+
+
+def offdiag_skip_bounds(pm: PackedModel, B: int, flags: int):
+  Mp = (pm.M + _lib.MM_M_ALIGN - 1) // _lib.MM_M_ALIGN * _lib.MM_M_ALIGN
+  Po = pm.L * (pm.L - 1) // 2 if (flags & MM_FULL_OUTPUT_COV) else 0
+  zt2s = torch.zeros(pm.L, Mp // 32, dtype=torch.float32, device=pm.device)
+  gmax2s = torch.zeros(B, Po, Mp // 64, dtype=torch.float32, device=pm.device)
+  ws = pm.workspace(B, flags, peek=True)
+  rc = lib().mm_offdiag_skip_bounds(pm.buf.data_ptr(), pm.nbytes, pm.L, pm.M, pm.d, _dtype_code(pm.dtype), B, flags,
+                                    ws.data_ptr(), ws.numel(), zt2s.data_ptr(), gmax2s.data_ptr(), _stream(pm.device))
+  check(rc, "mm_offdiag_skip_bounds")
+  return zt2s, gmax2s
 
 
 def route_estimates(pm: PackedModel, B: int, flags: int) -> torch.Tensor:
diff --git a/include/gpflowpilco_mm.h b/include/gpflowpilco_mm.h
--- a/include/gpflowpilco_mm.h
+++ b/include/gpflowpilco_mm.h
@@ -87,6 +87,12 @@
 
 int mm_offdiag_stats(const void* packed, size_t packed_bytes, int L, int M, int d, int dtype, int B, int flags,
                      const void* workspace, size_t workspace_bytes, int32_t* out, void* stream);
+
+int mm_offdiag_worklist_len(int L, int M, int d, int dtype, int B, int flags, const void* workspace, size_t workspace_bytes,
+                            int32_t* out, void* stream);
+
+int mm_offdiag_skip_bounds(const void* packed, size_t packed_bytes, int L, int M, int d, int dtype, int B, int flags,
+                           const void* workspace, size_t workspace_bytes, float* zt2s_out, float* gmax2s_out, void* stream);
 
 int mm_route_estimates(const void* packed, size_t packed_bytes, int L, int M, int d, int dtype, int B, int flags,
                        const void* workspace, size_t workspace_bytes, double* out, void* stream);
```

Measured after the change: 45210 rollout step-elements/s (B*H per rollout second) (median of 6 runs). 3.9% higher.
